# wwang2/CoarseGrainingVAE

Hardware: AMD Instinct MI355X
Metric: train_step_frames_per_sec (higher is better)
Workload: dtype f32

## Files before the change

### coarsegrainingvae_amd/_lib.py

```python
from __future__ import annotations

import ctypes as C
import os
import re
import threading

import torch

from . import ktimer

_PKG = os.path.dirname(os.path.abspath(__file__))
LIB_PATH = os.environ.get("CGV_LIB") or os.path.join(_PKG, "libcgvae_hip.so")
HEADER_PATH = os.path.join(os.path.dirname(_PKG), "include", "cgvae_hip.h")

_lock = threading.Lock()
_lib = None

_p, _i, _f, _sz = C.c_void_p, C.c_int, C.c_float, C.c_size_t

PROTOTYPES = {
    "cgv_version": (_i, []),
    "cgv_last_error_string": (C.c_char_p, []),
    "cgv_timestamp": (_i, [_p, _p]),
    "cgv_timestamp_hz": (_i, []),
# ... 17 lines not shown
    "cgv_edge_geometry_grouped": (_i, [_p, _p, _p, _p, _p, _i, _i, _f, _p, _p, _p]),
    "cgv_edge_geometry": (_i, [_p, _p, _p, _p, _p, _p, _i, _i, _f, _p, _p, _p]),
    "cgv_plan_jobs_max": (_i, []),
    "cgv_plan_job_bytes": (_i, []),
    "cgv_plan_jobs_build": (_i, [_p, _i, _p]),
    "cgv_geom_jobs_max": (_i, []),
    "cgv_geom_job_bytes": (_i, []),
    "cgv_geom_jobs_build": (_i, [_p, _i, _p]),
    "cgv_segment_reduce": (_i, [_p, _p, _p, _i, _i, _i, _p, _p]),
    "cgv_embedding_rows": (_i, [_p, _p, _i, _i, _i, _i, _p, _p]),
    "cgv_embedding_rows2": (_i, [_p, _p, _i, _i, _i, _p, _p, _p, _i, _i, _i, _p, _i, _p]),
    "cgv_segment_reduce_pair": (_i, [_p, _p, _p, _i, _p, _p, _p, _p, _i, _p, _i, _p]),
    "cgv_segment_broadcast": (_i, [_p, _p, _p, _i, _i, _i, _p, _p]),
    "cgv_equi_msg_fwd": (_i, [_p, _p, _p, _p, _p, _p, _p, _p, _p, _i, _i, _i, _i, C.c_int64, C.c_int64, _p, _p, _p]),
    "cgv_equi_msg_grouped_supported": (_i, [_i, _i, _i]),
    "cgv_equi_msg_fwd_grouped": (_i, [_p] * 9 + [_i, _i, _i, _i, C.c_int64, C.c_int64, _p, _p, _p]),
    "cgv_equi_msg_bwd_workspace_bytes": (_sz, [_i, _i, _i]),
    "cgv_equi_msg_bwd": (_i, [_p] * 13 + [_i, _i, _i, C.c_int64, C.c_int64, _p, _sz, _p]),
    "cgv_pseudo_msg_fwd": (_i, [_p] * 14 + [_i, _i, _i, _i, _p]),
    "cgv_pseudo_msg_fwd_rows": (_i, [_p] * 15 + [_i, _i, _i, _i, C.c_int64, _p]),
    "cgv_pseudo_msg_bwd_workspace_bytes": (_sz, [_i, _i, _i]),
    "cgv_pseudo_msg_bwd": (_i, [_p] * 24 + [_i, _i, _i, _i, C.c_int64, _p, _sz, _p]),
    "cgv_pseudo_msg_bwd_deferred": (_i, [_p] * 22 + [_i, _i, _i, _i, C.c_int64, _p, _sz, _p, _p]),
    "cgv_update_rows_from_vec": (_i, [_p, _p, _i, _i, _p]),
    "cgv_tile_bwd_input_plan": (_i, [_i, _i, _i, _i, _p, _p]),
    "cgv_tile_linear_bwd_input_norm_stack": (_i, [_p, _p, _p, _i, _i, _i, _i, _p, _p, _p, _p, _p, _i, _i, _p]),
    "cgv_update_vec_from_rows": (_i, [_p, _p, _p, _i, _i, _p]),
    "cgv_update_norm_stack_fwd": (_i, [_p, _p, _p, _i, _i, _i, _p]),
    "cgv_update_norm_stack_bwd": (_i, [_p, _p, _p, _p, _p, _p, _i, _i, _i, _i, _p]),
    "cgv_update_gate_fwd": (_i, [_p, _p, _p, _p, _p, _p, _p, _i, _i, _i, _p]),
    "cgv_update_gate_bwd": (_i, [_p, _p, _p, _p, _p, _p, _p, _p, _i, _i, _i, _p]),
    "cgv_skinny_max_rows": (_i, []),
    "cgv_skinny_supported": (_i, [_i, _i, _i]),
    "cgv_skinny_fwd_supported": (_i, [_i, _i, _i]),
    "cgv_skinny_linear_fwd": (_i, [_p, _p, _p, _p, _p, _i, _i, _i, _i, _p]),
    "cgv_skinny_bwd_input_supported": (_i, [_i, _i, _i]),
    "cgv_skinny_bwd_input_workspace_bytes": (_sz, [_i, _i, _i]),
    "cgv_skinny_linear_bwd_input": (_i, [_p, _p, _p, _p, _i, _i, _i, _i, _p, _sz, _p]),
    "cgv_decoder_layer_supported": (_i, [_i, _i, _i]),
    "cgv_decoder_slice_floats": (C.c_int64, [_i, _i]),
    "cgv_batch_load_rows": (_i, [_p, _p, _p, _i, _p, _p, _p, _i, _p]),
    "cgv_reparam_sample": (_i, [_p, _p, _p, _p, C.c_int64, _p, _p]),
    "cgv_reparam_bwd": (_i, [_p, _p, _p, _p, _p, _p, C.c_int64, _p]),
    "cgv_pair_linear_fwd": (_i, [_p] * 10 + [_i] * 5 + [_p]),
    "cgv_equi_msg_bwd_deferred": (_i, [_p] * 11 + [_i, _i, _i, C.c_int64, C.c_int64, _p, C.c_size_t, _p, _p, _p]),
    "cgv_filter_reduce_jobs_max": (_i, []),
    "cgv_filter_reduce_job_bytes": (_i, []),
    "cgv_filter_reduce_jobs": (_i, [_p, _i, _p]),
    "cgv_pair_linear_bwd_input": (_i, [_p] * 6 + [_i, _i, _p, _p, _i, _i, _i, _p, C.c_size_t, _p]),
    "cgv_loss_tail_supported": (_i, [_i, _i, _i, _i]),
    "cgv_loss_tail_workspace_bytes": (_sz, [_i]),
    "cgv_loss_tail": (_i, [_p] * 12 + [_i, _i, _i, _i, _i, _f, _f] + [_p] * 9 + [_p, _sz, _p]),
    "cgv_multi_linear_max": (_i, []),
    "cgv_multi_linear_fwd": (_i, [_i] + [_p] * 6 + [_i, _i, _i, _p]),
    "cgv_multi_linear_bwd_input": (_i, [_i, _i] + [_p] * 5 + [_i, _i, _i, _p, C.c_size_t, _p]),
    "cgv_decoder_max_edges": (_i, []),
    "cgv_decoder_block_channels": (_i, [_i]),
    "cgv_decoder_debug_clock": (_i, [_p]),
    "cgv_decoder_msg_fwd": (_i, [_p] * 18 + [_i, _i, _i, _i, _p]),
    "cgv_decoder_dense_fwd": (_i, [_p, _p, _p, _p, _p, _i, _i, _i, _i, _p]),
    "cgv_prior_msg_fwd": (_i, [_p] * 13 + [_i, _i, _i, _i, _i, _p]),
    "cgv_prior_msg_bwd": (_i, [_p] * 8 + [_i, C.c_int64] + [_p] * 6 + [C.c_int64, _i, _i, _i, _i, _p]),
    "cgv_decoder_uv_fwd": (_i, [_p, _p, _p, _p, _i, _i, _p]),
    "cgv_decoder_gate_fwd": (_i, [_p] * 9 + [_i, _i, _p]),
    "cgv_decoder_gate_bwd": (_i, [_p, _p, _p, _p, _i, C.c_int64, _p, _p, _p, _p, _p, _p, C.c_int64, _i, _i, _p]),
    "cgv_decoder_dense_bwd": (_i, [_p, _i, C.c_int64, _p, _i, _p, _p, _p, C.c_int64, _i, _i, _i, _p]),
    "cgv_decoder_uv_bwd": (_i, [_p, _i, C.c_int64, _p, _p, _p, _p, _p, _p, _p, _p, C.c_int64, _i, _i, _p]),
    "cgv_decoder_msg_bwd": (_i, [_p] * 15 + [_p, _i, C.c_int64, _p, _p, _p] + [_p] * 8 + [C.c_int64, _i, _i, _i, _i, _p]),
    "cgv_decoder_slices_to_dense": (_i, [_p, _p, _i, C.c_int64, _p, _i, _i, _p]),
    "cgv_dense_grad_prepare": (_i, [_p, _p, _p, _p, _i, _i, _i, _i, _p]),
    "cgv_tile_supported": (_i, [_i, _i, _i]),
    "cgv_tile_linear_fwd": (_i, [_p, _p, _p, _p, _p, _i, _i, _i, _i, _p]),
    "cgv_tile_linear_bwd_input": (_i, [_p, _p, _p, _i, _i, _i, _p]),
    "cgv_tile_linear_bwd_input_act": (_i, [_p, _p, _p, _p, _i, _i, _i, _i, _p]),
    "cgv_tile_linear_bwd_input_act_add": (_i, [_p, _p, _p, _p, _p, _i, _i, _i, _i, _p]),
    "cgv_tile_linear_bwd_input_act_add_bcast": (_i, [_p] * 7 + [_i, _p, _i, _i, _i, _i, _p]),
    "cgv_tile_pair_supported": (_i, [_i, _i, _i]),
    "cgv_tile_pair_linear_fwd": (_i, [_p] * 10 + [_i, _i, _i, _i, _i, _p]),
    "cgv_tile_pair_linear_bwd_input": (_i, [_p] * 10 + [_i, _i, _i, _i, _i, _p]),
    "cgv_tile_linear_bwd_input_out": (_i, [_p] * 5 + [_i, _i, _i, _i, _p, _i, _p]),
    "cgv_tile_bwd_input_split": (_i, [_p, _sz, _p]),
    "cgv_tile_pair_linear_bwd_input_out": (_i, [_p] * 10 + [_i, _i, _i, _i, _i, _p, _i, _p, _i, _p]),
    "cgv_tile_linear_bwd_input_sum2": (_i, [_p] * 10 + [_i, _p, _i, _i, _i, _i, _i, _p]),
    "cgv_segment_reduce2": (_i, [_p, _i, _p, _p, _i, _p, _p, _p, _i, _i, _p]),
    "cgv_skinny_linear_bwd_input_add": (_i, [_p, _p, _p, _p, _p, _i, _i, _i, _i, _p, _sz, _p]),
    "cgv_skinny_linear_bwd_input_out": (_i, [_p] * 5 + [_i, _i, _i, _i, _p, _i, _p, _sz, _p]),
    "cgv_tile_linear_wgrad": (_i, [_p, _p, _p, _i, _i, _i, _i, _p]),
    "cgv_wgrad_record_bytes": (_i, []),
    "cgv_wgrad_plan": (_i, [_i, _i, _i, _p, _p, _p]),
    "cgv_wgrad_lds_floats": (_i, [_i, _i]),
    "cgv_grouped_wgrad": (_i, [_p, _i, _i, _i, _p]),
    "cgv_wgrad_gathered_plan": (_i, [_i, _i, _i, _i, _p, _p]),
    "cgv_grouped_wgrad_gathered": (_i, [_p, _i, _i, _p]),
    "cgv_wgrad_gathered_plan_tile": (_i, [_i, _i, _i, _i, _i, _p, _p]),
    "cgv_grouped_wgrad_gathered_tile": (_i, [_p, _i, _i, _i, _p]),
    "cgv_grouped_wgrad_split": (_i, [_p, _i, _i, _p]),
    "cgv_grouped_wgrad_gathered_sumsq": (_i, [_p, _i, _i, _p, _p, _p]),
    "cgv_grouped_wgrad_gathered_adam": (_i, [_p, _i, _i, _p, _p, _p, _p, _f, _f, _f, _f, _p, _p]),
    "cgv_wgrad_strip_max_rows": (_i, []),
    "cgv_wgrad_strip_plan": (_i, [_i, _i, _i, _i, _p]),
    "cgv_wgrad_strip_split_max_rows": (_i, []),
    "cgv_wgrad_strip_split_plane_bytes": (_sz, [_i, _i]),
    "cgv_grouped_wgrad_strip_split": (_i, [_p, _i, _i, _i, _i, _p, _sz, _p]),
    "cgv_grouped_wgrad_strip": (_i, [_p, _i, _i, _i, _p]),
    "cgv_grouped_wgrad_strip_sumsq": (_i, [_p, _i, _i, _i, _p, _p, _p]),
    "cgv_grouped_wgrad_strip_adam": (_i, [_p, _i, _i, _i, _p, _p, _p, _p, _f, _f, _f, _f, _p, _p]),
    "cgv_pack_record_bytes": (_i, []),
    "cgv_pack_plan": (_i, [_i, _i, _i, _p]),
    "cgv_pack_operands": (_i, [_p, _i, _i, _p]),
    "cgv_reconstruct_fwd": (_i, [_p, _p, _p, _p, _p, _i, _i, _i, _p, _p]),
    "cgv_reconstruct_bwd": (_i, [_p, _p, _p, _p, _i, _i, _i, _p, _p, _p]),
    "cgv_elbo_workspace_bytes": (_sz, [_i, _i]),
    "cgv_elbo_fwd": (_i, [_p] * 7 + [_i, _i, _i, _i, _f, _f] + [_p] * 7 + [_p, _sz, _p]),
    "cgv_elbo_scale": (_i, [_p, _p, _p, _p, _p, _i, _p, _i, _p]),
    "cgv_optim_state_floats": (_i, []),
    "cgv_optim_partial_floats": (_i, []),
    "cgv_adam_clip_step": (_i, [_p, _p, _p, _p, C.c_int64, _f, _f, _f, _f, _f, _f, _p, _f, _p, _p, _p]),
    "cgv_optim_prepare": (_i, [_p, C.c_int64, _f, _f, _f, _f, _p, _f, _p, _p, _p]),
    "cgv_adam_apply": (_i, [_p, _p, _p, _p, C.c_int64, _f, _f, _f, _f, _p, _p]),
    "cgv_sgd_apply": (_i, [_p, _p, C.c_int64, _f, _p, _p]),
    "cgv_wgrad_gram": (_i, [_p, _i, _i, _p, _p, C.c_size_t, _p]),
    "cgv_wgrad_gram_workspace_bytes": (C.c_size_t, [_i]),
    "cgv_wgrad_gram_mfma": (_i, [_p, _i, _i, _p, _p, C.c_size_t, _p]),
    "cgv_wgrad_gram_mfma_workspace_bytes": (C.c_size_t, [_i, _i]),
    "cgv_wgrad_gram_mfma_max_rows": (_i, []),
    "cgv_rank_update_supported": (_i, [_i, _i, _i]),
    "cgv_optim_prepare_extra": (_i, [_p, C.c_int64, _p, _i, _f, _f, _f, _f, _p, _f, _p, _p, _p]),
    "cgv_grouped_wgrad_adam": (_i, [_p, _i, _i, _i, _p, _p, _p, _p, _f, _f, _f, _f, _p, _p]),
    "cgv_rank_flat_quantum": (_i, []),
    "cgv_rank_flat_plan": (_i, [_i, _i, _i, _i, _p, _p]),
    "cgv_grouped_wgrad_adam_flat": (_i, [_p, _i, _i, _i, _i, _p, _p, _p, _p, _f, _f, _f, _f, _p, _p]),
    "cgv_grouped_wgrad_adam_mixed": (_i, [_p, _i, _i, _i, _i, _i, _i, _p, _p, _p, _p, _f, _f, _f, _f, _p, _p]),
    "cgv_sample_quality_max_classes": (_i, []),
    "cgv_sample_quality": (_i, [_p] * 6 + [_i] * 5 + [_p, _p, _p]),
    "cgv_ensemble_check_max_classes": (_i, []),
    "cgv_ensemble_check_max_samples": (_i, []),
    "cgv_ensemble_check": (_i, [_p] * 7 + [_i] * 6 + [_p, _p, _p]),
    "cgv_internal_hist_max_features": (_i, []),
    "cgv_internal_hist_max_pairs": (_i, []),
    "cgv_internal_hist_max_bins": (_i, []),
    "cgv_internal_hist_max_bins2": (_i, []),
    "cgv_internal_hist_max_atoms": (_i, []),
    "cgv_internal_hist_max_staged_atoms": (_i, []),
    "cgv_internal_hist_feature_tile": (_i, [_i]),
    "cgv_internal_hist_pair_tile": (_i, [_i]),
    "cgv_internal_hist": (_i, [_p] * 4 + [_i] * 6 + [C.c_double] * 2 + [_p] * 3),
    "cgv_internal_values": (_i, [_p] * 3 + [_i] * 3 + [_p] * 3),
    "cgv_kde_max_planes": (_i, []),
    "cgv_kde_max_samples": (_i, []),
    "cgv_kde_max_points": (_i, []),
    "cgv_kde_max_splits": (_i, []),
    "cgv_kde_splits": (_i, [_i, _i, _i]),
    "cgv_kde_workspace_bytes": (_sz, [_i, _i, _i]),
    "cgv_kde_sums": (_i, [_p] * 3 + [_i] * 5 + [_p, _p, _p, _sz, _p]),
    "cgv_tica_max_features": (_i, []),
    "cgv_tica_max_atoms": (_i, []),
    "cgv_tica_max_bins2": (_i, []),
    "cgv_tica_max_components": (_i, []),
    "cgv_tica_moments_splits": (_i, [_i, _i, _i]),
    "cgv_tica_moments_workspace_bytes": (_sz, [_i, _i, _i]),
    "cgv_tica_moments": (_i, [_p, _p, _i, _i, _i, _i] + [_p] * 5 + [_p, _sz, _p]),
    "cgv_tica_project": (_i, [_p] * 4 + [_i] * 4 + [_p, _i, _i, _i] + [C.c_double] * 4 + [_p] * 3),
    "cgv_superpose_max_structures": (_i, []),
    "cgv_superpose_max_atoms": (_i, []),
    "cgv_superpose_workspace_bytes": (_sz, [_i, _i]),
    "cgv_superpose": (_i, [_p, _p, _p] + [_i] * 7 + [_p] * 5 + [_p, _sz, _p]),
# ... 108 lines not shown


def load():
    global _lib
    if _lib is not None:
        return _lib
    with _lock:
        if _lib is not None:
            return _lib
        if not os.path.exists(LIB_PATH):
            raise RuntimeError(
                f"{LIB_PATH} is missing: build it with `python -m coarsegrainingvae_amd.build` "
                "(hipcc --offload-arch=gfx950).  There is no fallback path.")
        lib = C.CDLL(LIB_PATH)
        for name, (res, args) in PROTOTYPES.items():
            fn = getattr(lib, name)
            fn.restype = res
            fn.argtypes = args
        if lib.cgv_version() < 101:
            raise RuntimeError("libcgvae_hip.so is older than this package")
        _lib = lib
    return _lib


def stream_ptr() -> int:
    return torch.cuda.current_stream().cuda_stream


def ptr(t):
    if t is None:
        return None
    if not t.is_cuda:
        raise RuntimeError("coarsegrainingvae_amd kernels need device (hip) tensors; there is no CPU path")
    if not t.is_contiguous():
        raise RuntimeError("tensor handed to the C ABI must be contiguous")
    return t.data_ptr()


_SPLIT_WS = {}
_SPLIT_TLS = threading.local()
_SPLIT_BYTES = 64 * 1024 + 64 * 1024 * 1024


def prepare_split_workspace(stream=None):
    st = torch.cuda.current_stream() if stream is None else stream
    key = (st.device.index if st.device.index is not None else torch.cuda.current_device(), int(st.cuda_stream))
    if key not in _SPLIT_WS:
        if torch.cuda.is_current_stream_capturing():
            return None
        _SPLIT_WS[key] = torch.zeros(_SPLIT_BYTES, dtype=torch.uint8, device=f"cuda:{key[0]}")
    return _SPLIT_WS[key]


def split_workspace_ready() -> bool:
    if load().cgv_get_option(OPTIONS["bwd_input_split"]) == 1:
        return False
    key = (torch.cuda.current_device(), int(torch.cuda.current_stream().cuda_stream))
    return key in _SPLIT_WS or not torch.cuda.is_current_stream_capturing()


def _register_split_workspace(lib):
    key = (torch.cuda.current_device(), int(torch.cuda.current_stream().cuda_stream))
    if getattr(_SPLIT_TLS, "cur", None) == key:
        return
    ws = prepare_split_workspace()
    if ws is None:
        lib.cgv_tile_bwd_input_split(None, 0, key[1])
        _SPLIT_TLS.cur = None
        return
    if lib.cgv_tile_bwd_input_split(ws.data_ptr(), ws.numel(), key[1]) != 0:
        raise RuntimeError("cgv_tile_bwd_input_split failed: " + lib.cgv_last_error_string().decode("utf-8", "replace"))
    _SPLIT_TLS.cur = key


def call(name: str, *args, tag=None):
    lib = load()
    if name.startswith("cgv_tile_") and ("bwd_input" in name or "linear_fwd" in name):
        _register_split_workspace(lib)
    tok = ktimer.begin(tag) if tag is not None else None
    rc = getattr(lib, name)(*args)
    ktimer.end(tok)
    if rc != 0:
        msg = lib.cgv_last_error_string().decode("utf-8", "replace")
        raise RuntimeError(f"{name} failed with code {rc}: {msg}")
```

### coarsegrainingvae_amd/csrc/tile_gemm.hip

```cpp
#include <stdlib.h>
#include <initializer_list>
#include <type_traits>
#include "cgv_common.h"
#include "streamk_gemm.h"

namespace cgv {

typedef float f32x4 __attribute__((ext_vector_type(4)));

__device__ __forceinline__ float4 ld4z(const float* p, bool ok) {
  return ok ? *reinterpret_cast<const float4*>(p) : make_float4(0.f, 0.f, 0.f, 0.f);
}

#define CGV_MFMA(a, b, c) __builtin_amdgcn_mfma_f32_16x16x4f32((a), (b), (c), 0, 0, 0)

template <int I0, int N, typename F>
__device__ __forceinline__ void static_for(F&& f) {
  if constexpr (I0 < N) {
    f(std::integral_constant<int, I0>{});
    static_for<I0 + 1, N>(f);
  }
}

struct TileSecond { const float* x; const float* W; const float* bias; float* y; float* z; int act; };
// ... 298 lines not shown
  __shared__ __attribute__((aligned(16))) float As[2][LT * LLD];
  __shared__ __attribute__((aligned(16))) float Bs[2][LT * LLD];
  const int t = threadIdx.x, lane = t & 63;
  const int wave = __builtin_amdgcn_readfirstlane(t >> 6);
  const int i = lane & 15, q = lane >> 4;
  const int wm = wave >> 1, wn = wave & 1;
  const int m0 = blockIdx.y * LT, n0 = blockIdx.x * LT;
  const int sr = t >> 3, sc = 4 * (t & 7);
  const float* const xr0 = x + (size_t)min(m0 + sr, M - 1) * K + sc;
  const float* const xr1 = x + (size_t)min(m0 + sr + 32, M - 1) * K + sc;
  const float* const wr0 = W + (size_t)min(n0 + sr, N - 1) * K + sc;
  const float* const wr1 = W + (size_t)min(n0 + sr + 32, N - 1) * K + sc;
  auto fetch = [&](RingSlot& r, int kt) __attribute__((always_inline)) {
    const int k0 = kt * LBK;
    const int off = (k0 + sc < K) ? k0 : -sc;
    r.a0 = *reinterpret_cast<const f32x4*>(xr0 + off); r.a1 = *reinterpret_cast<const f32x4*>(xr1 + off);
    r.b0 = *reinterpret_cast<const f32x4*>(wr0 + off); r.b1 = *reinterpret_cast<const f32x4*>(wr1 + off);
  };
  auto stash = [&](const RingSlot& r, int kt, int buf) __attribute__((always_inline)) {
    const bool kok = kt * LBK + sc < K;
    *reinterpret_cast<f32x4*>(&As[buf][sr * LLD + sc]) = r.a0;
    *reinterpret_cast<f32x4*>(&As[buf][(sr + 32) * LLD + sc]) = r.a1;
    *reinterpret_cast<f32x4*>(&Bs[buf][sr * LLD + sc]) = kok ? r.b0 : f32x4{0.f, 0.f, 0.f, 0.f};
    *reinterpret_cast<f32x4*>(&Bs[buf][(sr + 32) * LLD + sc]) = kok ? r.b1 : f32x4{0.f, 0.f, 0.f, 0.f};
  };
  RingSlot s0, s1, s2;
  fetch(s0, 0);
  fetch(s1, SLABS > 1 ? 1 : 0);
  fetch(s2, SLABS > 2 ? 2 : 0);
  f32x4 acc00 = {0.f, 0.f, 0.f, 0.f}, acc01 = acc00, acc10 = acc00, acc11 = acc00;
  stash(s0, 0, 0);
  __syncthreads();
#pragma unroll
  for (int kt = 0; kt < SLABS; ++kt) {
    const int buf = kt & 1;
    if (kt + 3 < SLABS) {
      switch (kt % 3) { case 0: fetch(s0, kt + 3); break; case 1: fetch(s1, kt + 3); break; default: fetch(s2, kt + 3); break; }
    }
    const float* __restrict__ a_s = As[buf] + (32 * wm + i) * LLD + 4 * q;
    const float* __restrict__ b_s = Bs[buf] + (32 * wn + i) * LLD + 4 * q;
#pragma unroll
    for (int ks = 0; ks < LBK / 16; ++ks) {
      const float4 x0 = *reinterpret_cast<const float4*>(a_s + 16 * ks), x1 = *reinterpret_cast<const float4*>(a_s + 16 * LLD + 16 * ks);
      const float4 w0 = *reinterpret_cast<const float4*>(b_s + 16 * ks), w1 = *reinterpret_cast<const float4*>(b_s + 16 * LLD + 16 * ks);
      acc00 = CGV_MFMA(w0.x, x0.x, acc00); acc01 = CGV_MFMA(w0.x, x1.x, acc01);
      acc10 = CGV_MFMA(w1.x, x0.x, acc10); acc11 = CGV_MFMA(w1.x, x1.x, acc11);
      acc00 = CGV_MFMA(w0.y, x0.y, acc00); acc01 = CGV_MFMA(w0.y, x1.y, acc01);
      acc10 = CGV_MFMA(w1.y, x0.y, acc10); acc11 = CGV_MFMA(w1.y, x1.y, acc11);
      acc00 = CGV_MFMA(w0.z, x0.z, acc00); acc01 = CGV_MFMA(w0.z, x1.z, acc01);
      acc10 = CGV_MFMA(w1.z, x0.z, acc10); acc11 = CGV_MFMA(w1.z, x1.z, acc11);
      acc00 = CGV_MFMA(w0.w, x0.w, acc00); acc01 = CGV_MFMA(w0.w, x1.w, acc01);
      acc10 = CGV_MFMA(w1.w, x0.w, acc10); acc11 = CGV_MFMA(w1.w, x1.w, acc11);
    }
    if (kt + 1 < SLABS) {
      switch ((kt + 1) % 3) { case 0: stash(s0, kt + 1, buf ^ 1); break; case 1: stash(s1, kt + 1, buf ^ 1); break; default: stash(s2, kt + 1, buf ^ 1); break; }
      __syncthreads();
    }
  }
  const f32x4 acc[2][2] = {{acc00, acc01}, {acc10, acc11}};
#pragma unroll
  for (int a = 0; a < 2; ++a) {
    const int n = n0 + 32 * wn + 16 * a + 4 * q;
    if (n >= N) continue;
    const float4 bv = bias ? *reinterpret_cast<const float4*>(bias + n) : make_float4(0.f, 0.f, 0.f, 0.f);
#pragma unroll
    for (int b = 0; b < 2; ++b) {
      const int m = m0 + 32 * wm + 16 * b + i;
      if (m >= M) continue;
      float4 zv = make_float4(acc[a][b][0] + bv.x, acc[a][b][1] + bv.y, acc[a][b][2] + bv.z, acc[a][b][3] + bv.w);
      if (act) {
        if (zout) *reinterpret_cast<float4*>(zout + (size_t)m * N + n) = zv;
        zv.x = act_fwd(zv.x, act); zv.y = act_fwd(zv.y, act); zv.z = act_fwd(zv.z, act); zv.w = act_fwd(zv.w, act);
      }
      *reinterpret_cast<float4*>(y + (size_t)m * N + n) = zv;
    }
  }
}

struct BwdSource { const float* g; const float* W; const float* z; int act; };
struct BwdSecond { const float* g; const float* W; float* gx; const float* z; const float* add; int act; };
struct OutAct { const float* z; int act; const float* z2; int act2; };
struct SplitN { float* part; unsigned* ticket; int n; };
struct NormStackOut { const float* stack; const float* Vv; const float* g_res; float* g_s; float* gVv; int F; int ld; int accumulate; };
struct BcastAdd {
  const float* src;
  const int64_t* row2seg;
  const int* rowptr;
  int mean;
};

#ifndef CGV_BWD_INPUT_PIPELINE
#define CGV_BWD_INPUT_PIPELINE 0
#endif
template <int MB, int WAVES>
__global__ __launch_bounds__(64 * WAVES) void tile_bwd_input_k(const float* __restrict__ g, const float* __restrict__ W,
                                                        float* __restrict__ gx, int M, int N, int K,
                                                        const float* __restrict__ z, int act,
                                                        const float* __restrict__ add = nullptr,
                                                        BcastAdd bc = BcastAdd{nullptr, nullptr, nullptr, 0},
                                                        BwdSecond s2 = BwdSecond{nullptr, nullptr, nullptr, nullptr, nullptr, 0},
                                                        BwdSource more = BwdSource{nullptr, nullptr, nullptr, 0},
                                                        OutAct oa = OutAct{nullptr, 0, nullptr, 0},
                                                        SplitN sp = SplitN{nullptr, nullptr, 1},
                                                        NormStackOut ns = NormStackOut{nullptr, nullptr, nullptr, nullptr, nullptr, 0, 0, 0}) {
  if (blockIdx.z) { g = s2.g; W = s2.W; gx = s2.gx; z = s2.z; add = s2.add; act = s2.act; bc.src = nullptr; oa.z = oa.z2; oa.act = oa.act2; }
  __shared__ float red[WAVES][MB * 4][4][64];
  const int lane = threadIdx.x & 63;
  const int wave = __builtin_amdgcn_readfirstlane(threadIdx.x >> 6);
  const int j = lane & 15, q = lane >> 4;
  const int ry = (int)blockIdx.y / sp.n, zs = (int)blockIdx.y - ry * sp.n;
  const int k0 = blockIdx.x * 64, m0 = ry * (16 * MB);
  const int kcol = k0 + 4 * j;
  const bool kok = kcol < K;
  const float* gr[MB];
  bool gok[MB];
#pragma unroll
  for (int mb = 0; mb < MB; ++mb) {
    const int m = m0 + 16 * mb + j;
    gok[mb] = m < M;
    gr[mb] = g + (size_t)(gok[mb] ? m : 0) * N + 4 * q;
  }
  const ptrdiff_t zoff = act ? z - g : 0;
  f32x4 acc[MB][4];
#pragma unroll
  for (int mb = 0; mb < MB; ++mb)
#pragma unroll
    for (int s = 0; s < 4; ++s) acc[mb][s] = f32x4{0.f, 0.f, 0.f, 0.f};
  const int steps_all = (N + 15) / 16, zper = (steps_all + sp.n - 1) / sp.n;
  const int z_beg = min(zs * zper, steps_all), steps = min(z_beg + zper, steps_all);
  const int per = (steps - z_beg + WAVES - 1) / WAVES;
  const int st_beg = min(z_beg + wave * per, steps), st_end = min(st_beg + per, steps);
  constexpr int SB = WAVES >= 16 ? 3 : 2;
  const float* wcol = W + (kok ? kcol : 0);
  ptrdiff_t zo = zoff;
  const int n_src = more.g ? 2 : 1;
  for (int src = 0; src < n_src; ++src) {
  if (src == 1) {
#pragma unroll
    for (int mb = 0; mb < MB; ++mb) gr[mb] = more.g + (gr[mb] - g);
    act = more.act;
    zo = act ? more.z - more.g : 0;
    wcol = more.W + (kok ? kcol : 0);
  }
  struct Batch { float4 a[SB][MB], zz[SB][MB], b[SB][4]; };
  auto request = [&](Batch& B, int st0) __attribute__((always_inline)) {
#pragma unroll
    for (int u = 0; u < SB; ++u) {
      const int n = 16 * (st0 + u);
      const bool in = st0 + u < st_end && n + 4 * q < N;
      const int ng = in ? n : -4 * q, nw = in ? n + 4 * q : 0;
#pragma unroll
      for (int mb = 0; mb < MB; ++mb) {
        B.a[u][mb] = *reinterpret_cast<const float4*>(gr[mb] + ng);
        if (act) B.zz[u][mb] = *reinterpret_cast<const float4*>(gr[mb] + zo + ng);
      }
#pragma unroll
      for (int c = 0; c < 4; ++c) B.b[u][c] = *reinterpret_cast<const float4*>(wcol + (size_t)(nw + c) * K);
    }
  };
  auto multiply = [&](const Batch& B, int st0) __attribute__((always_inline)) {
#pragma unroll
    for (int u = 0; u < SB; ++u) {
      if (st0 + u >= st_end) break;
      const bool nok = 16 * (st0 + u) + 4 * q < N;
#pragma unroll
      for (int mb = 0; mb < MB; ++mb) {
        float4 av = B.a[u][mb];
        if (act) {
          av.x *= act_bwd(B.zz[u][mb].x, act); av.y *= act_bwd(B.zz[u][mb].y, act);
          av.z *= act_bwd(B.zz[u][mb].z, act); av.w *= act_bwd(B.zz[u][mb].w, act);
        }
        const float ac[4] = {nok ? av.x : 0.f, nok ? av.y : 0.f, nok ? av.z : 0.f, nok ? av.w : 0.f};
#pragma unroll
        for (int c = 0; c < 4; ++c) {
          acc[mb][0] = CGV_MFMA(ac[c], B.b[u][c].x, acc[mb][0]);
          acc[mb][1] = CGV_MFMA(ac[c], B.b[u][c].y, acc[mb][1]);
          acc[mb][2] = CGV_MFMA(ac[c], B.b[u][c].z, acc[mb][2]);
          acc[mb][3] = CGV_MFMA(ac[c], B.b[u][c].w, acc[mb][3]);
        }
      }
    }
  };
  if constexpr (CGV_BWD_INPUT_PIPELINE && WAVES < 16) {
    Batch b0, b1;
    int st0 = st_beg;
    request(b0, st0);
    for (; st0 < st_end; st0 += 2 * SB) {
      request(b1, st0 + SB);
      multiply(b0, st0);
      request(b0, st0 + 2 * SB);
      multiply(b1, st0 + SB);
    }
  } else {
    for (int st0 = st_beg; st0 < st_end; st0 += SB) {
      Batch b0;
      request(b0, st0);
      multiply(b0, st0);
    }
  }
  }
  constexpr int PAIRS = MB * 4, PER = (PAIRS + WAVES - 1) / WAVES;
  float4 pre_add[PER], pre_z[PER];
  if (kok && (add || oa.z)) {
#pragma unroll
    for (int u = 0; u < PER; ++u) {
      const int c = wave + u * WAVES;
      if (c < PAIRS) {
        const size_t at = (size_t)min(m0 + 16 * (c >> 2) + 4 * q + (c & 3), M - 1) * K + kcol;
        if (add) pre_add[u] = *reinterpret_cast<const float4*>(add + at);
        if (oa.z) pre_z[u] = *reinterpret_cast<const float4*>(oa.z + at);
      }
    }
  }
#pragma unroll
  for (int t = 0; t < MB * 4; ++t)
#pragma unroll
    for (int r = 0; r < 4; ++r) red[wave][t][r][lane] = acc[t >> 2][t & 3][r];
  __syncthreads();
  float* tile_part = nullptr;
  if (sp.n > 1) {
    unsigned* s_last = reinterpret_cast<unsigned*>(&red[0][0][0][0]);
    const size_t tid = ((size_t)blockIdx.z * (gridDim.y / sp.n) + ry) * gridDim.x + blockIdx.x;
    tile_part = sp.part + tid * sp.n * (size_t)(MB * 16 * 64);
#pragma unroll
    for (int u = 0; u < PER; ++u) {
      const int c = wave + u * WAVES;
      if (c >= PAIRS) break;
      const int mb = c >> 2, r = c & 3;
      f32x4 o;
#pragma unroll
      for (int sI = 0; sI < 4; ++sI) {
        const int t = mb * 4 + sI;
        float a = red[0][t][r][lane];
#pragma unroll
        for (int w = 1; w < WAVES; ++w) a += red[w][t][r][lane];
        o[sI] = a;
      }
      float* dst = tile_part + (size_t)zs * (MB * 16 * 64) + (16 * mb + 4 * q + r) * 64 + 4 * j;
      asm volatile("global_store_dwordx4 %0, %1, off sc1" : : "v"(dst), "v"(o) : "memory");
    }
    asm volatile("s_waitcnt vmcnt(0)" ::: "memory");
    __syncthreads();
    if (threadIdx.x == 0) *s_last = atomicAdd(sp.ticket + tid, 1u) == (unsigned)(sp.n - 1) ? 1u : 0u;
    __syncthreads();
    if (!*s_last) return;
    if (threadIdx.x == 0) __hip_atomic_store(sp.ticket + tid, 0u, __ATOMIC_RELAXED, __HIP_MEMORY_SCOPE_AGENT);
  }
// ... 201 lines not shown
                       act);
  else if (lds_min == 5)
    hipLaunchKernelGGL((cgv::tile_fwd_k<1, 2, 8>), dim3((N + 63) / 64, (M + 31) / 32), dim3(1024), 0, st, x, W, bias, y, z, M, N, K, act);
  else if (lds_min == 6)
    hipLaunchKernelGGL((cgv::tile_fwd_k<2, 1, 8>), dim3((N + 31) / 32, (M + 63) / 64), dim3(1024), 0, st, x, W, bias, y, z, M, N, K, act);
  else if (lds_min == 7)
    hipLaunchKernelGGL((cgv::tile_fwd_k<2, 2, 4>), dim3((N + 63) / 64, (M + 63) / 64), dim3(1024), 0, st, x, W, bias, y, z, M, N, K, act);
  else if (tiles32 >= 2048)
    hipLaunchKernelGGL((cgv::tile_fwd_k<2, 2, 4>), dim3((N + 63) / 64, (M + 63) / 64, np), dim3(1024), 0, st, x, W, bias, y, z, M,
                       N, K, act, s2);
  else
    hipLaunchKernelGGL((cgv::tile_fwd_k<1, 1, 8>), dim3((N + 31) / 32, (M + 31) / 32, np), dim3(512), 0, st, x, W, bias, y, z, M,
                       N, K, act, s2);
  return cgv::check_launch("cgv_tile_linear_fwd");
}

int cgv_tile_linear_fwd(const float* x, const float* W, const float* bias, float* y, float* z, int M, int N, int K, int act,
                        void* stream) {
  CGV_REQUIRE(x && W && y, "null pointer");
  CGV_REQUIRE(act >= 0 && act <= cgv::CGV_ACT_MAX, "act must be 0 (identity), 1 (swish), 2 (tanh), 3 (relu), 4 / 5 (c + exp(z/2))");
  CGV_REQUIRE(cgv_tile_supported(M, N, K), "unsupported shape (need N % 4 == 0, K % 4 == 0)");
  CGV_REQUIRE(((((uintptr_t)x | (uintptr_t)W)) & 15) == 0, "x and W must be 16-byte aligned");
  return tile_fwd_launch(x, W, bias, y, z, M, N, K, act, stream, nullptr);
}

int cgv_tile_pair_supported(int M, int N, int K) {
  return cgv_tile_supported(M, N, K);
}

int cgv_tile_pair_linear_fwd(const float* x_a, const float* W_a, const float* bias_a, float* y_a, float* z_a, const float* x_b,
                             const float* W_b, const float* bias_b, float* y_b, float* z_b, int M, int N, int K, int act_a,
                             int act_b, void* stream) {
  const int act = act_a;
  CGV_REQUIRE(x_a && W_a && y_a && x_b && W_b && y_b, "null pointer");
  CGV_REQUIRE(act_a >= 0 && act_a <= cgv::CGV_ACT_MAX && act_b >= 0 && act_b <= cgv::CGV_ACT_MAX,
              "act must be 0 (identity), 1 (swish), 2 (tanh), 3 (relu), 4 / 5 (c + exp(z/2))");
  CGV_REQUIRE((act_a == 0 || z_a) && (act_b == 0 || z_b), "act != 0 needs the pre-activation output");
  CGV_REQUIRE(cgv_tile_supported(M, N, K), "unsupported shape (need N % 4 == 0, K % 4 == 0)");
  CGV_REQUIRE(((((uintptr_t)x_a | (uintptr_t)W_a | (uintptr_t)x_b | (uintptr_t)W_b | (uintptr_t)y_a | (uintptr_t)y_b |
                 (uintptr_t)z_a | (uintptr_t)z_b | (uintptr_t)bias_a | (uintptr_t)bias_b)) & 15) == 0, "operands must be 16-byte aligned");
  const cgv::TileSecond s2{x_b, W_b, bias_b, y_b, z_b, act_b};
  return tile_fwd_launch(x_a, W_a, bias_a, y_a, z_a, M, N, K, act, stream, &s2);
}


static int split_shares(int tiles, int N) {
  const int opt = cgv::option(CGV_OPT_BWD_INPUT_SPLIT);
  if (opt == 1 || tiles > 128 || tiles < 1) return 1;
  int n = opt >= 2 ? opt : 256 / tiles;
  n = n > 4 ? 4 : n;
  while (n > 1 && (N + 15) / 16 / n < 16) --n;
  return n < 1 ? 1 : n;
}

namespace cgv {
enum BwdKernel { BWD_R16_W8, BWD_R16_W16, BWD_R32_W8, BWD_R32_W4 };
struct BwdInputChoice {
  int bpc;
  BwdKernel kernel;
  int shares;
};

static BwdInputChoice bwd_input_choice(int M, int N, int K, int np, bool ws) {
  BwdInputChoice c{ws ? sk_wanted(M, K, N, np) : 0, BWD_R16_W8, 1};
  const int kt = (K + 63) / 64;
  const int blocks32 = kt * ((M + 31) / 32);
  const int blocks16 = kt * ((M + 15) / 16);
  const int ow = option(CGV_OPT_BWD_INPUT_WAVES);
  int waves = 8;
  if (ow > 0 && ow != 32) waves = ow;
  else if (blocks16 < 128 && N >= 1024) waves = 16;
  if (ow == 32 || (blocks32 >= 200 && blocks32 < 512 && waves == 8))
    c.kernel = BWD_R32_W8;
  else if (blocks32 >= 512)
    c.kernel = BWD_R32_W4;
  else if (waves == 16) {
    c.kernel = BWD_R16_W16;
    if (ws) c.shares = split_shares(blocks16 * np, N);
  }
  return c;
}
}

static int tile_bwd_input_launch(const float* g, const float* z, int act, const float* W, float* gx, int M, int N, int K,
                                 void* stream, const char* what, const float* add = nullptr,
                                 cgv::BcastAdd bc = cgv::BcastAdd{nullptr, nullptr, nullptr, 0},
                                 const cgv::BwdSecond* second = nullptr,
                                 cgv::BwdSource more = cgv::BwdSource{nullptr, nullptr, nullptr, 0},
                                 cgv::OutAct oa = cgv::OutAct{nullptr, 0, nullptr, 0},
                                 cgv::NormStackOut ns = cgv::NormStackOut{nullptr, nullptr, nullptr, nullptr, nullptr, 0, 0, 0}) {
  hipStream_t st = (hipStream_t)stream;
  const cgv::BwdSecond s2 = second ? *second : cgv::BwdSecond{nullptr, nullptr, nullptr, nullptr, nullptr, 0};
  const unsigned np = second ? 2u : 1u;
  const cgv::BwdInputChoice choice = cgv::bwd_input_choice(M, N, K, (int)np, cgv::sk_ws_ready(stream));
  if (const int bpc = choice.bpc;
      bpc != 0 && !ns.stack && act == 0 && (!more.g || more.act == 0) && (!second || s2.act == 0) &&
      cgv::sk_aligned({g, W, gx, add, bc.src, more.g, more.W, oa.z, oa.z2, s2.g, s2.W, s2.gx, s2.add})) {
    cgv::SkArgs a{};
    a.np = (int)np; a.M = M; a.N = K;
    cgv::SkProblem& p0 = a.p[0];
    p0.A[0] = g; p0.B[0] = W; p0.R[0] = N; p0.out = gx; p0.add = add;
    if (more.g) { p0.A[1] = more.g; p0.B[1] = more.W; p0.R[1] = N; }
    p0.bc_src = bc.src; p0.bc_row2seg = bc.row2seg; p0.bc_rowptr = bc.rowptr; p0.bc_mean = bc.mean;
    p0.oz = oa.z; p0.oact = oa.act;
    if (second) {
      cgv::SkProblem& p1 = a.p[1];
      p1.A[0] = s2.g; p1.B[0] = s2.W; p1.R[0] = N; p1.out = s2.gx; p1.add = s2.add; p1.oz = oa.z2; p1.oact = oa.act2;
    }
    if (cgv::sk_launch(a, true, cgv::g_split_ws.ws, cgv::g_split_ws.bytes, cgv::SPLIT_TICKET_BYTES, st, bpc) == 0)
      return cgv::check_launch(what);
  }
  const int kt = (K + 63) / 64;
  switch (choice.kernel) {
    case cgv::BWD_R32_W8:
      hipLaunchKernelGGL((cgv::tile_bwd_input_k<2, 8>), dim3(kt, (M + 31) / 32, np), dim3(512), 0, st, g, W, gx, M, N, K, z, act, add, bc, s2, more, oa, cgv::SplitN{nullptr, nullptr, 1}, ns);
      break;
    case cgv::BWD_R32_W4:
      hipLaunchKernelGGL((cgv::tile_bwd_input_k<2, 4>), dim3(kt, (M + 31) / 32, np), dim3(256), 0, st, g, W, gx, M, N, K, z, act, add, bc, s2, more, oa, cgv::SplitN{nullptr, nullptr, 1}, ns);
      break;
    case cgv::BWD_R16_W16: {
      cgv::SplitN sp{nullptr, nullptr, 1};
      const int tiles = kt * ((M + 15) / 16) * (int)np;
      const cgv::SplitWs& w = cgv::g_split_ws;
      const size_t need = cgv::SPLIT_TICKET_BYTES + (size_t)tiles * choice.shares * (16 * 64) * sizeof(float);
      if (choice.shares > 1 && need <= w.bytes && (size_t)tiles * sizeof(unsigned) <= cgv::SPLIT_TICKET_BYTES) {
        sp.ticket = reinterpret_cast<unsigned*>(w.ws);
        sp.part = reinterpret_cast<float*>(reinterpret_cast<char*>(w.ws) + cgv::SPLIT_TICKET_BYTES);
        sp.n = choice.shares;
      }
      hipLaunchKernelGGL((cgv::tile_bwd_input_k<1, 16>), dim3(kt, ((M + 15) / 16) * sp.n, np), dim3(1024), 0, st, g, W, gx, M, N, K, z, act,
                         add, bc, s2, more, oa, sp, ns);
      break;
    }
    case cgv::BWD_R16_W8:
      hipLaunchKernelGGL((cgv::tile_bwd_input_k<1, 8>), dim3(kt, (M + 15) / 16, np), dim3(512), 0, st, g, W, gx, M, N, K, z, act, add, bc, s2, more, oa, cgv::SplitN{nullptr, nullptr, 1}, ns);
      break;
  }
  return cgv::check_launch(what);
}

int cgv_tile_bwd_input_plan(int M, int N, int K, int np, int* shares, int* streamk) {
  CGV_REQUIRE(shares && streamk && np >= 1 && np <= 2, "bad argument");
  CGV_REQUIRE(cgv_tile_supported(M, N, K), "unsupported shape (need N % 4 == 0, K % 4 == 0)");
  const cgv::BwdInputChoice c = cgv::bwd_input_choice(M, N, K, np, true);
  *streamk = c.bpc != 0;
  *shares = c.bpc != 0 ? 1 : c.shares;
  return 0;
}

int cgv_tile_bwd_input_split(void* ws, size_t bytes, void* stream) {
  CGV_REQUIRE(!ws || ((((uintptr_t)ws) & 15) == 0 && bytes >= cgv::SPLIT_TICKET_BYTES + (2u << 20)), "workspace too small / misaligned");
  cgv::g_split_ws = cgv::SplitWs{ws, ws ? bytes : 0, stream};
  return 0;
}

int cgv_tile_linear_bwd_input(const float* g, const float* W, float* gx, int M, int N, int K, void* stream) {
  CGV_REQUIRE(g && W && gx, "null pointer");
  CGV_REQUIRE(cgv_tile_supported(M, N, K), "unsupported shape (need N % 4 == 0, K % 4 == 0)");
  CGV_REQUIRE(((((uintptr_t)g | (uintptr_t)W | (uintptr_t)gx)) & 15) == 0, "g, W and gx must be 16-byte aligned");
  return tile_bwd_input_launch(g, nullptr, 0, W, gx, M, N, K, stream, "cgv_tile_linear_bwd_input");
}

int cgv_tile_linear_bwd_input_act(const float* gy, const float* z, const float* W, float* gx, int M, int N, int K, int act,
                                  void* stream) {
  CGV_REQUIRE(gy && W && gx, "null pointer");
  CGV_REQUIRE(act == 0 || (act >= 1 && act <= cgv::CGV_ACT_MAX && z), "act != 0 needs the saved pre-activation z");
  CGV_REQUIRE(cgv_tile_supported(M, N, K), "unsupported shape (need N % 4 == 0, K % 4 == 0)");
  CGV_REQUIRE(((((uintptr_t)gy | (uintptr_t)z | (uintptr_t)W | (uintptr_t)gx)) & 15) == 0, "operands must be 16-byte aligned");
  return tile_bwd_input_launch(gy, act ? z : nullptr, act, W, gx, M, N, K, stream, "cgv_tile_linear_bwd_input_act");
}

int cgv_tile_linear_bwd_input_act_add(const float* gy, const float* z, const float* W, const float* add, float* gx, int M, int N,
                                      int K, int act, void* stream) {
  CGV_REQUIRE(gy && W && gx && add, "null pointer");
  CGV_REQUIRE(act == 0 || (act >= 1 && act <= cgv::CGV_ACT_MAX && z), "act != 0 needs the saved pre-activation z");
  CGV_REQUIRE(cgv_tile_supported(M, N, K), "unsupported shape (need N % 4 == 0, K % 4 == 0)");
  CGV_REQUIRE(((((uintptr_t)gy | (uintptr_t)z | (uintptr_t)W | (uintptr_t)gx | (uintptr_t)add)) & 15) == 0, "operands must be 16-byte aligned");
  return tile_bwd_input_launch(gy, act ? z : nullptr, act, W, gx, M, N, K, stream, "cgv_tile_linear_bwd_input_act_add", add);
}

int cgv_tile_linear_bwd_input_act_add_bcast(const float* gy, const float* z, const float* W, const float* add, const float* seg_grad,
                                            const int64_t* row2seg, const int32_t* seg_rowptr, int mean, float* gx, int M, int N,
                                            int K, int act, void* stream) {
  CGV_REQUIRE(gy && W && gx && seg_grad && row2seg && seg_rowptr, "null pointer");
  CGV_REQUIRE(act == 0 || (act >= 1 && act <= cgv::CGV_ACT_MAX && z), "act != 0 needs the saved pre-activation z");
  CGV_REQUIRE(cgv_tile_supported(M, N, K), "unsupported shape (need N % 4 == 0, K % 4 == 0)");
  CGV_REQUIRE(((((uintptr_t)gy | (uintptr_t)z | (uintptr_t)W | (uintptr_t)gx | (uintptr_t)add | (uintptr_t)seg_grad)) & 15) == 0,
              "operands must be 16-byte aligned");
  return tile_bwd_input_launch(gy, act ? z : nullptr, act, W, gx, M, N, K, stream, "cgv_tile_linear_bwd_input_act_add_bcast", add,
                               cgv::BcastAdd{seg_grad, row2seg, seg_rowptr, mean});
}

int cgv_tile_linear_bwd_input_sum2(const float* gy_a, const float* z_a, const float* W_a, const float* gy_b, const float* z_b,
                                   const float* W_b, const float* add, const float* seg_grad, const int64_t* row2seg,
                                   const int32_t* seg_rowptr, int mean, float* gx, int M, int N, int K, int act_a, int act_b,
                                   void* stream) {
  CGV_REQUIRE(gy_a && W_a && gy_b && W_b && gx, "null pointer");
  CGV_REQUIRE((act_a == 0 || (act_a >= 1 && act_a <= cgv::CGV_ACT_MAX && z_a)) && (act_b == 0 || (act_b >= 1 && act_b <= cgv::CGV_ACT_MAX && z_b)),
              "act != 0 needs the saved pre-activation");
  CGV_REQUIRE(!seg_grad || (row2seg && seg_rowptr), "seg_grad needs its row -> segment map and the segments' row pointers");
  CGV_REQUIRE(cgv_tile_supported(M, N, K), "unsupported shape (need N % 4 == 0, K % 4 == 0)");
  CGV_REQUIRE(((((uintptr_t)gy_a | (uintptr_t)z_a | (uintptr_t)W_a | (uintptr_t)gy_b | (uintptr_t)z_b | (uintptr_t)W_b | (uintptr_t)gx |
                 (uintptr_t)add | (uintptr_t)seg_grad)) & 15) == 0, "operands must be 16-byte aligned");
  return tile_bwd_input_launch(gy_a, act_a ? z_a : nullptr, act_a, W_a, gx, M, N, K, stream, "cgv_tile_linear_bwd_input_sum2", add,
                               cgv::BcastAdd{seg_grad, row2seg, seg_rowptr, mean}, nullptr,
                               cgv::BwdSource{gy_b, W_b, act_b ? z_b : nullptr, act_b});
}

int cgv_tile_pair_linear_bwd_input(const float* gy_a, const float* z_a, const float* W_a, const float* add_a, float* gx_a,
                                   const float* gy_b, const float* z_b, const float* W_b, const float* add_b, float* gx_b, int M,
                                   int N, int K, int act_a, int act_b, void* stream) {
  const int act = act_a;
  CGV_REQUIRE(gy_a && W_a && gx_a && gy_b && W_b && gx_b && gx_a != gx_b, "null pointer / aliased outputs");
  CGV_REQUIRE((act_a == 0 || (act_a >= 1 && act_a <= cgv::CGV_ACT_MAX && z_a)) && (act_b == 0 || (act_b >= 1 && act_b <= cgv::CGV_ACT_MAX && z_b)),
              "act != 0 needs the saved pre-activation");
  CGV_REQUIRE(cgv_tile_supported(M, N, K), "unsupported shape (need N % 4 == 0, K % 4 == 0)");
  CGV_REQUIRE(((((uintptr_t)gy_a | (uintptr_t)z_a | (uintptr_t)W_a | (uintptr_t)gx_a | (uintptr_t)add_a | (uintptr_t)gy_b |
                 (uintptr_t)z_b | (uintptr_t)W_b | (uintptr_t)gx_b | (uintptr_t)add_b)) & 15) == 0, "operands must be 16-byte aligned");
  const cgv::BwdSecond s2{gy_b, W_b, gx_b, act_b ? z_b : nullptr, add_b, act_b};
  return tile_bwd_input_launch(gy_a, act ? z_a : nullptr, act, W_a, gx_a, M, N, K, stream, "cgv_tile_pair_linear_bwd_input", add_a,
                               cgv::BcastAdd{nullptr, nullptr, nullptr, 0}, &s2);
}

int cgv_tile_linear_bwd_input_out(const float* gy, const float* z, const float* W, const float* add, float* gx, int M, int N,
                                  int K, int act, const float* z_out, int act_out, void* stream) {
  CGV_REQUIRE(gy && W && gx && z_out, "null pointer");
  CGV_REQUIRE(act == 0 || (act >= 1 && act <= cgv::CGV_ACT_MAX && z), "act != 0 needs the saved pre-activation z");
  CGV_REQUIRE(act_out >= 1 && act_out <= cgv::CGV_ACT_MAX, "act_out must name an activation");
  CGV_REQUIRE(cgv_tile_supported(M, N, K), "unsupported shape (need N % 4 == 0, K % 4 == 0)");
  CGV_REQUIRE(((((uintptr_t)gy | (uintptr_t)z | (uintptr_t)W | (uintptr_t)gx | (uintptr_t)add | (uintptr_t)z_out)) & 15) == 0,
              "operands must be 16-byte aligned");
  return tile_bwd_input_launch(gy, act ? z : nullptr, act, W, gx, M, N, K, stream, "cgv_tile_linear_bwd_input_out", add,
                               cgv::BcastAdd{nullptr, nullptr, nullptr, 0}, nullptr, cgv::BwdSource{nullptr, nullptr, nullptr, 0},
                               cgv::OutAct{z_out, act_out, nullptr, 0});
}

int cgv_tile_linear_bwd_input_norm_stack(const float* gy, const float* z, const float* W, int M, int N, int K, int act,
                                         const float* stack, const float* Vv, const float* g_res, float* g_s, float* gVv, int ld,
                                         int accumulate, void* stream) {
  CGV_REQUIRE(gy && W && stack && Vv && g_s && gVv, "null pointer");
  CGV_REQUIRE(act == 0 || (act >= 1 && act <= cgv::CGV_ACT_MAX && z), "act != 0 needs the saved pre-activation z");
  CGV_REQUIRE(cgv_tile_supported(M, N, K) && K % 8 == 0 && ld >= K / 2 && ld % 4 == 0, "unsupported shape (need K = 2 F, F % 4 == 0, ld % 4 == 0)");
  CGV_REQUIRE(((((uintptr_t)gy | (uintptr_t)z | (uintptr_t)W | (uintptr_t)stack | (uintptr_t)Vv | (uintptr_t)g_res | (uintptr_t)g_s |
                 (uintptr_t)gVv)) & 15) == 0, "operands must be 16-byte aligned");
  return tile_bwd_input_launch(gy, act ? z : nullptr, act, W, g_s , M, N, K, stream,
                               "cgv_tile_linear_bwd_input_norm_stack", nullptr, cgv::BcastAdd{nullptr, nullptr, nullptr, 0}, nullptr,
                               cgv::BwdSource{nullptr, nullptr, nullptr, 0}, cgv::OutAct{nullptr, 0, nullptr, 0},
                               cgv::NormStackOut{stack, Vv, g_res, g_s, gVv, K / 2, ld, accumulate});
}

int cgv_tile_pair_linear_bwd_input_out(const float* gy_a, const float* z_a, const float* W_a, const float* add_a, float* gx_a,
                                       const float* gy_b, const float* z_b, const float* W_b, const float* add_b, float* gx_b,
                                       int M, int N, int K, int act_a, int act_b, const float* z_out_a, int act_out_a,
                                       const float* z_out_b, int act_out_b, void* stream) {
  const int act = act_a;
  CGV_REQUIRE(gy_a && W_a && gx_a && gy_b && W_b && gx_b && gx_a != gx_b, "null pointer / aliased outputs");
  CGV_REQUIRE((act_a == 0 || (act_a >= 1 && act_a <= cgv::CGV_ACT_MAX && z_a)) && (act_b == 0 || (act_b >= 1 && act_b <= cgv::CGV_ACT_MAX && z_b)),
              "act != 0 needs the saved pre-activation");
  CGV_REQUIRE((!z_out_a || (act_out_a >= 1 && act_out_a <= cgv::CGV_ACT_MAX)) && (!z_out_b || (act_out_b >= 1 && act_out_b <= cgv::CGV_ACT_MAX)),
              "z_out needs its activation code");
  CGV_REQUIRE(cgv_tile_supported(M, N, K), "unsupported shape (need N % 4 == 0, K % 4 == 0)");
  CGV_REQUIRE(((((uintptr_t)gy_a | (uintptr_t)z_a | (uintptr_t)W_a | (uintptr_t)gx_a | (uintptr_t)add_a | (uintptr_t)gy_b |
                 (uintptr_t)z_b | (uintptr_t)W_b | (uintptr_t)gx_b | (uintptr_t)add_b | (uintptr_t)z_out_a | (uintptr_t)z_out_b)) & 15) == 0,
              "operands must be 16-byte aligned");
  const cgv::BwdSecond s2{gy_b, W_b, gx_b, act_b ? z_b : nullptr, add_b, act_b};
  return tile_bwd_input_launch(gy_a, act ? z_a : nullptr, act, W_a, gx_a, M, N, K, stream, "cgv_tile_pair_linear_bwd_input_out", add_a,
                               cgv::BcastAdd{nullptr, nullptr, nullptr, 0}, &s2, cgv::BwdSource{nullptr, nullptr, nullptr, 0},
                               cgv::OutAct{z_out_a, z_out_a ? act_out_a : 0, z_out_b, z_out_b ? act_out_b : 0});
}

int cgv_tile_linear_wgrad(const float* g, const float* x, float* gW, int M, int N, int K, int accumulate, void* stream) {
  CGV_REQUIRE(g && x && gW, "null pointer");
  CGV_REQUIRE(cgv_tile_supported(M, N, K), "unsupported shape (need N % 4 == 0, K % 4 == 0)");
  CGV_REQUIRE(((((uintptr_t)x | (uintptr_t)gW)) & 15) == 0, "x and gW must be 16-byte aligned");
  const dim3 grid((K + 63) / 64, (N + 15) / 16);
  if (grid.x * grid.y >= 1024 || M <= 128)
    hipLaunchKernelGGL((cgv::tile_wgrad_k<4>), grid, dim3(256), 0, (hipStream_t)stream, g, x, gW, M, N, K, accumulate);
  else
    hipLaunchKernelGGL((cgv::tile_wgrad_k<8>), grid, dim3(512), 0, (hipStream_t)stream, g, x, gW, M, N, K, accumulate);
  return cgv::check_launch("cgv_tile_linear_wgrad");
}

}
```

### coarsegrainingvae_amd/csrc/wgrad_gathered.hip

```cpp
#include "cgv_common.h"
#include "gemm_dev.h"
#include "wgrad_record.h"

namespace cgv {

__device__ __forceinline__ float4 ldg4_or_zero(const float* p, bool ok) {
  return ok ? *reinterpret_cast<const float4*>(p) : make_float4(0.f, 0.f, 0.f, 0.f);
}
__device__ __forceinline__ void strip_pin() { asm volatile("" ::: "memory"); }
typedef const float __attribute__((address_space(1)))* strip_gptr;
__device__ __forceinline__ float4 strip_ldg4(const float* p) {
  const f32x4 t = *reinterpret_cast<const __attribute__((address_space(1))) f32x4*>((strip_gptr)p);
  return make_float4(t.x, t.y, t.z, t.w);
}
#ifndef CGV_GW_CHUNK
#define CGV_GW_CHUNK 48
#endif
constexpr int GW_CHUNK = CGV_GW_CHUNK;
constexpr int GW_GS = 80, GW_XS = 64;
constexpr int GW_TW = 128, GW_XW = 128;

enum { GW_STORE = 0, GW_SUMSQ = 1, GW_ADAM = 2 };
template <int MODE>
__global__ __launch_bounds__(256) void gathered_wgrad_k(const WgradProblem* __restrict__ table, int n_problems,
// ... 433 lines not shown
#pragma unroll
    for (int p = 0; p < NP; ++p) {
      *reinterpret_cast<float4*>(gs + (rr + 8 * p) * GW2_GS + 4 * c4) = gq[p];
      *reinterpret_cast<float4*>(xs + (rr + 8 * p) * GW2_XS + 4 * c4) = xq[p];
    }
    __syncthreads();
    if (m0 + GW2_CHUNK < M) chunk_load(m0 + GW2_CHUNK);
    const int steps = (rows + 3) / 4;
#pragma unroll 2
    for (int st = 0; st < steps; ++st) {
      const float4 b = *reinterpret_cast<const float4*>(xs + (4 * st + q) * GW2_XS + 64 * wk + 4 * i);
#pragma unroll
      for (int t = 0; t < 4; ++t) {
        const float a = gs[(4 * st + q) * GW2_GS + 64 * wn + 16 * t + i];
        bsum[t] += a;
        acc[t][0] = __builtin_amdgcn_mfma_f32_16x16x4f32(a, b.x, acc[t][0], 0, 0, 0);
        acc[t][1] = __builtin_amdgcn_mfma_f32_16x16x4f32(a, b.y, acc[t][1], 0, 0, 0);
        acc[t][2] = __builtin_amdgcn_mfma_f32_16x16x4f32(a, b.z, acc[t][2], 0, 0, 0);
        acc[t][3] = __builtin_amdgcn_mfma_f32_16x16x4f32(a, b.w, acc[t][3], 0, 0, 0);
      }
    }
    __syncthreads();
  }
  const int kcol = k0 + 64 * wk + 4 * i;
  if (kcol < K) {
#pragma unroll
    for (int t = 0; t < 4; ++t)
#pragma unroll
      for (int r = 0; r < 4; ++r) {
        const int row = n0 + 64 * wn + 16 * t + 4 * q + r;
        if (row >= N) continue;
        float4* dst = reinterpret_cast<float4*>(pr.gW + (size_t)row * K + kcol);
        float4 o = make_float4(acc[t][0][r], acc[t][1][r], acc[t][2][r], acc[t][3][r]);
        if (pr.accumulate) { const float4 old = *dst; o.x += old.x; o.y += old.y; o.z += old.z; o.w += old.w; }
        *dst = o;
      }
  }
  if (pr.gb && kt == 0 && wk == 0) {
#pragma unroll
    for (int t = 0; t < 4; ++t) {
      float b = bsum[t];
      b += __shfl_xor(b, 16);
      b += __shfl_xor(b, 32);
      const int n = n0 + 64 * wn + 16 * t + i;
      if (q == 0 && n < N) pr.gb[n] = pr.accumulate ? pr.gb[n] + b : b;
    }
  }
}

typedef __bf16 sp_bf16x2 __attribute__((ext_vector_type(2)));
typedef __bf16 sp_bf16x8 __attribute__((ext_vector_type(8)));
typedef float sp_f32x2 __attribute__((ext_vector_type(2)));
constexpr int SP_CHUNK = 32;
constexpr int SP_LD = 40;

__device__ __forceinline__ void sp_split(float a, float b, unsigned& hi, unsigned& mid, unsigned& lo) {
  const sp_f32x2 v = {a, b};
  const sp_bf16x2 h = __builtin_convertvector(v, sp_bf16x2);
  const sp_f32x2 r = v - __builtin_convertvector(h, sp_f32x2);
  const sp_bf16x2 m = __builtin_convertvector(r, sp_bf16x2);
  const sp_f32x2 r2 = r - __builtin_convertvector(m, sp_f32x2);
  const sp_bf16x2 l = __builtin_convertvector(r2, sp_bf16x2);
  hi = __builtin_bit_cast(unsigned, h);
  mid = __builtin_bit_cast(unsigned, m);
  lo = __builtin_bit_cast(unsigned, l);
}
__device__ __forceinline__ void sp_store4(unsigned short* dst, int plane, float v0, float v1, float v2, float v3) {
  unsigned h0, m0, l0, h1, m1, l1;
  sp_split(v0, v1, h0, m0, l0);
  sp_split(v2, v3, h1, m1, l1);
  *reinterpret_cast<uint2*>(dst) = make_uint2(h0, h1);
  *reinterpret_cast<uint2*>(dst + plane) = make_uint2(m0, m1);
  *reinterpret_cast<uint2*>(dst + 2 * plane) = make_uint2(l0, l1);
}

__global__ __launch_bounds__(256, 2) void wgrad_split128_k(const WgradProblem* __restrict__ table, int n_problems) {
  constexpr int PLANE = 128 * SP_LD;
  __shared__ __attribute__((aligned(16))) unsigned short gs[3 * PLANE];
  __shared__ __attribute__((aligned(16))) unsigned short xs[3 * PLANE];
  const int item = blockIdx.x;
  const int lo = wg_find_problem(table, n_problems, item);
  const WgradProblem pr = table[lo];
  const int local = item - pr.block_begin;
  const int nb = local / pr.tiles_k, kt = local - nb * pr.tiles_k;
  const int M = pr.M, N = pr.N, K = pr.K;
  const int sr = pr.seg_rows > 0 ? pr.seg_rows : M;
  const int n0 = nb * 128, k0 = kt * 128;
  const int lane = threadIdx.x & 63;
  const int wave = __builtin_amdgcn_readfirstlane(threadIdx.x >> 6);
  const int wn = wave >> 1, wk = wave & 1;
  const int i = lane & 15, q = lane >> 4;
  typedef float f32x4 __attribute__((ext_vector_type(4)));
  f32x4 acc[4][4];
#pragma unroll
  for (int t = 0; t < 4; ++t)
#pragma unroll
    for (int c = 0; c < 4; ++c) acc[t][c] = f32x4{0.f, 0.f, 0.f, 0.f};
  const int c4 = 8 * wave + (lane & 7), rq = lane >> 3;
  const bool gcol = n0 + 4 * c4 < N, xcol = k0 + 4 * c4 < K;
  const int gcol_at = gcol ? n0 + 4 * c4 : 0, xcol_at = xcol ? k0 + 4 * c4 : 0;
  const float* zsrc = pr.act ? pr.z : pr.gy;
  float4 gq[4], zq[4], xq[4];
  float bs[4] = {0.f, 0.f, 0.f, 0.f};
  auto chunk_load = [&](int m0) {
#pragma unroll
    for (int r = 0; r < 4; ++r) {
      const int m = min(m0 + 4 * rq + r, M - 1);
      const int seg = m / sr, row = m - seg * sr;
      const size_t base = (size_t)seg * pr.seg_stride;
      gq[r] = strip_ldg4(pr.gy + base + (size_t)row * N + gcol_at);
      zq[r] = strip_ldg4(zsrc + base + (size_t)row * N + gcol_at);
      xq[r] = strip_ldg4(pr.x + base + (size_t)row * K + xcol_at);
    }
    strip_pin();
  };
  unsigned short* gdst = gs + (4 * c4) * SP_LD + 4 * rq;
  unsigned short* xdst = xs + (64 * (c4 >> 4) + (c4 & 15)) * SP_LD + 4 * rq;
  auto chunk_store = [&](int m0) {
    if (pr.act == 1) {
#pragma unroll
      for (int r = 0; r < 4; ++r) {
        gq[r].x *= act_bwd(zq[r].x, 1); gq[r].y *= act_bwd(zq[r].y, 1);
        gq[r].z *= act_bwd(zq[r].z, 1); gq[r].w *= act_bwd(zq[r].w, 1);
      }
    } else if (pr.act) {
#pragma unroll
      for (int r = 0; r < 4; ++r) {
        gq[r].x *= act_bwd(zq[r].x, pr.act); gq[r].y *= act_bwd(zq[r].y, pr.act);
        gq[r].z *= act_bwd(zq[r].z, pr.act); gq[r].w *= act_bwd(zq[r].w, pr.act);
      }
    }
#pragma unroll
    for (int r = 0; r < 4; ++r) {
      const bool live = m0 + 4 * rq + r < M;
      if (!(live && gcol)) gq[r] = make_float4(0.f, 0.f, 0.f, 0.f);
      if (!(live && xcol)) xq[r] = make_float4(0.f, 0.f, 0.f, 0.f);
    }
    bs[0] += (gq[0].x + gq[1].x) + (gq[2].x + gq[3].x);
    bs[1] += (gq[0].y + gq[1].y) + (gq[2].y + gq[3].y);
    bs[2] += (gq[0].z + gq[1].z) + (gq[2].z + gq[3].z);
    bs[3] += (gq[0].w + gq[1].w) + (gq[2].w + gq[3].w);
    sp_store4(gdst, PLANE, gq[0].x, gq[1].x, gq[2].x, gq[3].x);
    sp_store4(gdst + SP_LD, PLANE, gq[0].y, gq[1].y, gq[2].y, gq[3].y);
    sp_store4(gdst + 2 * SP_LD, PLANE, gq[0].z, gq[1].z, gq[2].z, gq[3].z);
    sp_store4(gdst + 3 * SP_LD, PLANE, gq[0].w, gq[1].w, gq[2].w, gq[3].w);
    sp_store4(xdst, PLANE, xq[0].x, xq[1].x, xq[2].x, xq[3].x);
    sp_store4(xdst + 16 * SP_LD, PLANE, xq[0].y, xq[1].y, xq[2].y, xq[3].y);
    sp_store4(xdst + 32 * SP_LD, PLANE, xq[0].z, xq[1].z, xq[2].z, xq[3].z);
    sp_store4(xdst + 48 * SP_LD, PLANE, xq[0].w, xq[1].w, xq[2].w, xq[3].w);
  };
  const unsigned short* ga = gs + (64 * wn + i) * SP_LD + 8 * q;
  const unsigned short* xb = xs + (64 * wk + i) * SP_LD + 8 * q;
  chunk_load(0);
  for (int m0 = 0; m0 < M; m0 += SP_CHUNK) {
    chunk_store(m0);
    __syncthreads();
    chunk_load(min(m0 + SP_CHUNK, M - 1));
    sp_bf16x8 a[3][4];
#pragma unroll
    for (int s = 0; s < 3; ++s)
#pragma unroll
      for (int t = 0; t < 4; ++t) a[s][t] = *reinterpret_cast<const sp_bf16x8*>(ga + s * PLANE + 16 * t * SP_LD);
#pragma unroll
    for (int c = 0; c < 4; ++c) {
      sp_bf16x8 b[3];
#pragma unroll
      for (int s = 0; s < 3; ++s) b[s] = *reinterpret_cast<const sp_bf16x8*>(xb + s * PLANE + 16 * c * SP_LD);
#pragma unroll
      for (int t = 0; t < 4; ++t) acc[t][c] = __builtin_amdgcn_mfma_f32_16x16x32_bf16(a[0][t], b[2], acc[t][c], 0, 0, 0);
#pragma unroll
      for (int t = 0; t < 4; ++t) acc[t][c] = __builtin_amdgcn_mfma_f32_16x16x32_bf16(a[2][t], b[0], acc[t][c], 0, 0, 0);
#pragma unroll
      for (int t = 0; t < 4; ++t) acc[t][c] = __builtin_amdgcn_mfma_f32_16x16x32_bf16(a[1][t], b[1], acc[t][c], 0, 0, 0);
#pragma unroll
      for (int t = 0; t < 4; ++t) acc[t][c] = __builtin_amdgcn_mfma_f32_16x16x32_bf16(a[0][t], b[1], acc[t][c], 0, 0, 0);
#pragma unroll
      for (int t = 0; t < 4; ++t) acc[t][c] = __builtin_amdgcn_mfma_f32_16x16x32_bf16(a[1][t], b[0], acc[t][c], 0, 0, 0);
#pragma unroll
      for (int t = 0; t < 4; ++t) acc[t][c] = __builtin_amdgcn_mfma_f32_16x16x32_bf16(a[0][t], b[0], acc[t][c], 0, 0, 0);
    }
    __syncthreads();
  }
  const int kcol = k0 + 64 * wk + 4 * i;
// ... 415 lines not shown
```

### coarsegrainingvae_amd/csrc/wgrad_record.h

```cpp
#pragma once
#include "cgv_common.h"

namespace cgv {

struct WgradProblem {
  const float* gy;
  const float* x;
  const float* z;
  float* gW;
  float* gb;
  int M, N, K;
  int accumulate, act;
  int block_begin;
  int tiles_k;
  int tile_w;
  int seg_rows;
  int seg_stride;
  int pad;
};
static_assert(sizeof(WgradProblem) == 88, "host/device record layout");
__device__ __forceinline__ size_t wg_row(const WgradProblem& pr, int m, int width) {
  if (pr.seg_rows <= 0) return (size_t)m * width;
  const int seg = m / pr.seg_rows;
  return (size_t)seg * pr.seg_stride + (size_t)(m - seg * pr.seg_rows) * width;
}

template <typename Problem>
__device__ __forceinline__ int wg_find_problem(const Problem* __restrict__ table, int n_problems, int block) {
  const int lane = threadIdx.x & 63;
  int count = 0;
  for (int base = 0; base < n_problems; base += 64) {
    const int i = base + lane;
    const int bb = i < n_problems ? table[i].block_begin : 0x7fffffff;
    count += __popcll(__ballot(bb <= block));
  }
  return __builtin_amdgcn_readfirstlane(count > 0 ? count - 1 : 0);
}
template <typename Problem>
__device__ __forceinline__ int wg_find_problem(const Problem* __restrict__ table, int n_problems) {
  return wg_find_problem(table, n_problems, (int)blockIdx.x);
}

struct RankUpdateArgs {
  const float* arena_g;
  float* arena_p;
  float* arena_m;
  float* arena_v;
  const float* state;
  float lr, beta1, beta2, eps;
};

constexpr int GRAM_MAX_ROWS = 64;

}
```

### coarsegrainingvae_amd/ops.py

```python
from __future__ import annotations

from typing import Optional

import ctypes as C
from types import SimpleNamespace

import torch

from . import _lib, options
from .graph import EdgeGeometry, EdgePlan
from .primitives import FWD_ENTRY, bwd_input_choice, bwd_input_launch, fwd_choice, linear as _linear, wgrad_queue, wgrad_sink

_F32 = torch.float32


def _c(t: Optional[torch.Tensor]) -> Optional[torch.Tensor]:
    if t is None:
        return None
    if t.dtype != _F32:
        raise RuntimeError("the HIP path computes in fp32 only")
    return t.contiguous()


def _filter_grad_targets(params, Wd, bd):
    pW, pb = params
    direct = all(getattr(p, "_cgv_direct", False) and p.grad is not None and p._cgv_pending and p.grad.is_contiguous()
                 for p in (pW, pb))
    if direct:
        pW._cgv_pending = pb._cgv_pending = False
        return pW.grad, pb.grad, None, None
    gWd, gbd = torch.empty_like(Wd), torch.empty_like(bd)
    return gWd, gbd, gWd, gbd


def _grouped_forward_usable(plan, geom, F, tensors8, Wd) -> bool:
    if not getattr(plan, "group_rb", 0) or getattr(geom, "geom_g", None) is None or plan.n_edges == 0:
        return False
    if not _lib.load().cgv_equi_msg_grouped_supported(F, geom.n_rbf, plan.group_rb):
        return False
    if plan.n_src * 12 * F >= 0x7fffffff or Wd.data_ptr() % 16:
        return False
    return all(t is None or t.data_ptr() % 8 == 0 for t in tensors8)


class _EquiMessage(torch.autograd.Function):

    @staticmethod
    def forward(ctx, phi, v, Wd, bd, plan: EdgePlan, geom: EdgeGeometry, with_dv: bool, s_res, v_res):
        filter_params = (Wd, bd)
        phi, v, Wd, bd, s_res, v_res = _c(phi), _c(v), _c(Wd), _c(bd), _c(s_res), _c(v_res)
        ctx.residual = (s_res is not None, v_res is not None)
        F = phi.shape[1] // 3
        if phi.shape[0] != plan.n_src or v.shape != (plan.n_src, F, 3) or Wd.shape != (3 * F, geom.n_rbf):
            raise RuntimeError("shape mismatch between node features, filter weights and the edge plan")
        ds = torch.empty(plan.n_dst, F, dtype=_F32, device=phi.device)
        if with_dv:
            dv = torch.empty(plan.n_dst, F, 3, dtype=_F32, device=phi.device)
        else:
            dv = v_res.clone() if v_res is not None else torch.zeros(plan.n_dst, F, 3, dtype=_F32, device=phi.device)
        tag = f"equi_msg_fwd:Nd{plan.n_dst}:E{plan.n_edges}:dv{int(with_dv)}"
        grouped = with_dv and _grouped_forward_usable(plan, geom, F, (phi, v, ds, dv, s_res, v_res, bd), Wd)
        if grouped:
            _lib.call("cgv_equi_msg_fwd_grouped", _lib.ptr(phi), _lib.ptr(v), _lib.ptr(geom.geom_g), _lib.ptr(plan.rowptr_d),
                      _lib.ptr(plan.src_g), _lib.ptr(Wd), _lib.ptr(bd), _lib.ptr(ds), _lib.ptr(dv),
                      plan.n_dst, F, geom.n_rbf, plan.group_rb, plan.n_src, plan.n_edges, _lib.ptr(s_res), _lib.ptr(v_res),
                      _lib.stream_ptr(), tag=tag)
        else:
            _lib.call("cgv_equi_msg_fwd", _lib.ptr(phi), _lib.ptr(v), _lib.ptr(geom.geom_d), _lib.ptr(plan.rowptr_d),
                      _lib.ptr(plan.src_d), _lib.ptr(Wd), _lib.ptr(bd), _lib.ptr(ds), _lib.ptr(dv), plan.n_dst, F,
                      geom.n_rbf, int(with_dv), plan.n_edges, plan.n_src, _lib.ptr(s_res), _lib.ptr(v_res),
                      _lib.stream_ptr(), tag=tag)
        ctx.save_for_backward(phi, v, Wd, bd)
        ctx.filter_params = filter_params
        ctx.plan, ctx.geom, ctx.with_dv = plan, geom, with_dv
        ctx.set_materialize_grads(False)
        return ds, dv

    @staticmethod
    def backward(ctx, gs, gv):
        phi, v, Wd, bd = ctx.saved_tensors
        plan, geom = ctx.plan, ctx.geom
        F = phi.shape[1] // 3
        dev = phi.device
        g_sres = gs if ctx.residual[0] else None
        g_vres = gv if ctx.residual[1] else None
        if not ctx.with_dv:
            gv = None
        if gs is None and gv is None:
            return (None,) * 7 + (g_sres, g_vres)
        gs, gv = _c(gs), _c(gv)
        g_phi = torch.empty_like(phi)
        g_v = torch.empty_like(v) if gv is not None else None
        gWd, gbd, ret_W, ret_b = _filter_grad_targets(ctx.filter_params, Wd, bd)
        lib = _lib.load()
        ws_bytes = int(lib.cgv_equi_msg_bwd_workspace_bytes(plan.n_src, F, geom.n_rbf))
        ws = torch.empty(ws_bytes, dtype=torch.uint8, device=dev)
        if wgrad_queue.active and ret_W is None and ret_b is None:
            nc, kl = C.c_int(), C.c_int()
            _lib.call("cgv_equi_msg_bwd_deferred", _lib.ptr(phi), _lib.ptr(v), _lib.ptr(geom.geom_s), _lib.ptr(plan.rowptr_s),
                      _lib.ptr(plan.dst_s), _lib.ptr(Wd), _lib.ptr(bd), _lib.ptr(gs), _lib.ptr(gv), _lib.ptr(g_phi), _lib.ptr(g_v),
                      plan.n_src, F, geom.n_rbf, plan.n_edges, plan.n_dst, _lib.ptr(ws), ws_bytes, C.byref(nc), C.byref(kl),
                      _lib.stream_ptr(), tag=f"equi_msg_bwd:Nd{plan.n_dst}:E{plan.n_edges}:gv{int(gv is not None)}")
            wgrad_queue.enqueue_filter(ws, nc.value, kl.value, geom.n_rbf, F, gWd, gbd)
            return g_phi, g_v, ret_W, ret_b, None, None, None, g_sres, g_vres
        _lib.call("cgv_equi_msg_bwd", _lib.ptr(phi), _lib.ptr(v), _lib.ptr(geom.geom_s), _lib.ptr(plan.rowptr_s),
                  _lib.ptr(plan.dst_s), _lib.ptr(Wd), _lib.ptr(bd), _lib.ptr(gs), _lib.ptr(gv), _lib.ptr(g_phi),
                  _lib.ptr(g_v), _lib.ptr(gWd), _lib.ptr(gbd), plan.n_src, F, geom.n_rbf, plan.n_edges, plan.n_dst, _lib.ptr(ws), ws_bytes,
                  _lib.stream_ptr(), tag=f"equi_msg_bwd:Nd{plan.n_dst}:E{plan.n_edges}:gv{int(gv is not None)}")
        return g_phi, g_v, ret_W, ret_b, None, None, None, g_sres, g_vres


def equi_message(phi, v, Wd, bd, plan: EdgePlan, geom: EdgeGeometry, with_dv: bool = True, s_res=None, v_res=None):
    return _EquiMessage.apply(phi, v, Wd, bd, plan, geom, with_dv, s_res, v_res)


class _SegmentReduce(torch.autograd.Function):
    @staticmethod
    def forward(ctx, src, plan: EdgePlan, mean: bool):
        src = _c(src)
        rows = src.shape[0]
        if rows != plan.n_edges:
            raise RuntimeError("index plan and src disagree on the number of rows")
        flat = src.reshape(rows, -1)
        C = flat.shape[1]
        out = torch.empty((plan.n_dst, C), dtype=_F32, device=src.device)
        _lib.call("cgv_segment_reduce", _lib.ptr(flat), _lib.ptr(plan.rowptr_d), _lib.ptr(plan.eid_d), plan.n_dst, C,
                  int(mean), _lib.ptr(out), _lib.stream_ptr())
        ctx.plan, ctx.mean, ctx.shape = plan, mean, tuple(src.shape)
        ctx.set_materialize_grads(False)
        return out.reshape((plan.n_dst,) + tuple(src.shape[1:]))

    @staticmethod
    def backward(ctx, gout):
        if gout is None:
            return None, None, None
        plan = ctx.plan
        gout = _c(gout).reshape(plan.n_dst, -1)
        C = gout.shape[1]
        gsrc = torch.empty((plan.n_edges, C), dtype=_F32, device=gout.device)
        _lib.call("cgv_segment_broadcast", _lib.ptr(gout), _lib.ptr(plan.rowptr_d), _lib.ptr(plan.eid_d), plan.n_dst,
                  C, int(ctx.mean), _lib.ptr(gsrc), _lib.stream_ptr())
        return gsrc.reshape(ctx.shape), None, None


class _Embedding(torch.autograd.Function):

    @staticmethod
    def forward(ctx, weight, idx, plan: EdgePlan):
        ctx.plan, ctx.param = plan, weight
        if idx.dtype == torch.float32 and idx.dim() == 1 and weight.shape[1] % 4 == 0:
            out = torch.empty(idx.shape[0], weight.shape[1], dtype=_F32, device=weight.device)
            _lib.call("cgv_embedding_rows", _lib.ptr(weight.detach()), idx.data_ptr(), int(idx.stride(0)), idx.shape[0],
                      weight.shape[0], weight.shape[1], _lib.ptr(out), _lib.stream_ptr())
            return out
        return weight.index_select(0, idx.long())

    @staticmethod
    def backward(ctx, g):
        from .primitives import _grad_target
        plan, w = ctx.plan, ctx.param
        g = _c(g)
        n_types, F = w.shape
        target, accumulate, ret = _grad_target(w, w)
        out = torch.empty_like(target) if accumulate else target
        _lib.call("cgv_segment_reduce", _lib.ptr(g), _lib.ptr(plan.rowptr_d), _lib.ptr(plan.eid_d), n_types, F, 0,
                  _lib.ptr(out), _lib.stream_ptr())
        if accumulate:
            target.add_(out)
        return ret, None, None


class _Embedding2(torch.autograd.Function):

    @staticmethod
    def forward(ctx, w_a, idx_a, plan_a, w_b, idx_b, plan_b):
        F = w_a.shape[1]
        out_a = torch.empty(idx_a.shape[0], F, dtype=_F32, device=w_a.device)
        out_b = torch.empty(idx_b.shape[0], F, dtype=_F32, device=w_a.device)
        _lib.call("cgv_embedding_rows2", _lib.ptr(w_a.detach()), idx_a.data_ptr(), int(idx_a.stride(0)), idx_a.shape[0], w_a.shape[0],
                  _lib.ptr(out_a), _lib.ptr(w_b.detach()), idx_b.data_ptr(), int(idx_b.stride(0)), idx_b.shape[0], w_b.shape[0],
                  _lib.ptr(out_b), F, _lib.stream_ptr())
        ctx.plans, ctx.params = (plan_a, plan_b), (w_a, w_b)
        ctx.set_materialize_grads(False)
        return out_a, out_b

    @staticmethod
# ... 661 lines not shown
```

### coarsegrainingvae_amd/options.py

```python
from __future__ import annotations

from . import _lib

HOST = {
    "fwd_group": -1,
    "wgrad_kernel": 0,
    "table_upload": 0,
    "wgrad_tile": 64,
    "rank_update": 1,
    "rank_flat": 2,
    "rank_mixed": 1,
    "rank_rows_mfma": -1,
    "rank_gram_rows": -1,
    "concurrent_prior": 0,
    "quad_heads": 1,
    "fused_loss_tail": 1,
    "paired_embeddings": 1,
    "pair_sum2": 1,
    "head_pairs": 1,
    "encoder_pairs": 1,
    "wgrad_split": 1,
    "fused_bead_mean": 1,
    "fused_prior": 1,
    "act_downstream": 1,
    "update_fused_bwd": 1,
    "strip_split": 1,
    "cgae_form": 0,
    "newman_form": 0,
    "baseline_form": 0,
    "align_form": 0,
    "kde_splits": 0,
    "decoder_dense": 0,
}
_DEFAULTS = dict(HOST)


def set(name: str, value: int) -> None:
    if name in HOST:
        HOST[name] = int(value)
    elif name in _lib.OPTIONS:
        _lib.set_option(name, int(value))
    else:
        raise KeyError(f"unknown option {name!r}; known: {sorted(HOST) + sorted(_lib.OPTIONS)}")


def get(name: str) -> int:
    return HOST[name] if name in HOST else _lib.get_option(name)


def reset() -> None:
    HOST.update(_DEFAULTS)
    _lib.reset_options()


def apply(specs) -> None:
    for spec in specs or ():
        name, _, value = spec.partition("=")
        set(name.strip(), int(value))


def pop_cli(argv) -> list:
    rest, i = [], 0
    while i < len(argv):
        if argv[i] == "--option" and i + 1 < len(argv):
            apply([argv[i + 1]])
            i += 2
        else:
            rest.append(argv[i])
            i += 1
    return rest
```

### coarsegrainingvae_amd/primitives.py

```python
from __future__ import annotations

import ctypes as C
import struct

import numpy as np
import torch
import torch.nn.functional as Fn
from torch import nn

from . import _lib


class Swish(nn.Module):

    def forward(self, x):
        return Fn.silu(x)


class shifted_softplus(nn.Module):
    def forward(self, x):
        return Fn.softplus(x) - np.log(2.0)


layer_types = {
    "linear": nn.Linear, "Tanh": nn.Tanh, "ReLU": nn.ReLU, "shifted_softplus": shifted_softplus,
    "sigmoid": nn.Sigmoid, "Dropout": nn.Dropout, "LeakyReLU": nn.LeakyReLU, "ELU": nn.ELU, "swish": Swish,
}


def to_module(activation: str) -> nn.Module:
    return layer_types[activation]()


def gemm_mode_or_none(x2, weight, bias):
    if not (x2.is_cuda and weight.is_cuda):
        return None, ("Dense / Linear run on the HIP kernels only: move the module and its input to the device "
                      "(there is no CPU / library fallback)")
    if x2.dtype != torch.float32 or weight.dtype != torch.float32:
        return None, "the HIP path computes in fp32 only"
    if not (weight.is_contiguous() and weight.data_ptr() % 16 == 0):
        return None, "Dense / Linear: the weight must be contiguous and 16-byte aligned"
    M, K = x2.shape
    N = weight.shape[0]
    if M == 0:
        return None, f"Dense / Linear on an input without rows (0 x {K})"
    lib = _lib.load()
    if lib.cgv_skinny_supported(M, N, K) and (bias is None or bias.data_ptr() % 16 == 0):
        return "skinny", None
    if lib.cgv_tile_supported(M, N, K):
        return "tile", None
    return None, (f"Dense / Linear {M} x {N} x {K}: the HIP kernels take in / out widths that are multiples of 4 "
                  f"(other widths are zero-padded by primitives.linear_fn before they get here)")


def _gemm_mode(x2, weight, bias):
    mode, why = gemm_mode_or_none(x2, weight, bias)
    if mode is None:
        raise RuntimeError(why)
    return mode


ACT_NONE, ACT_SWISH, ACT_TANH, ACT_RELU = 0, 1, 2, 3
ACT_STD_ENC, ACT_STD_PRIOR = 4, 5
_STD_EPS = {ACT_STD_ENC: 1e-12, ACT_STD_PRIOR: 1e-9}


class WeightGradQueue:

    RECORD = struct.Struct("<5Q11i4x")
    MAX_PROBLEMS = 512

    def __init__(self):
        self.active = False
        self.items = []
        self._captured = []
        self._capture_slots = []
        self._deferred = []
        self.filters = []

    @property
    def kernel(self):
        from .options import HOST
        return "mfma" if HOST["wgrad_kernel"] == 1 else "valu"

    @property
    def static_tables(self):
        from .options import HOST
        return HOST["table_upload"] != 1

    def prepare_capture(self, device, flushes: int = 4):
        n = self.MAX_PROBLEMS * self.RECORD.size
        self._captured = []
        self._capture_slots = [(torch.empty(n, dtype=torch.uint8).pin_memory(),
                                torch.empty(n, dtype=torch.uint8, device=device)) for _ in range(flushes)]

    def collect(self):
        return _QueueScope(self)

    def enqueue(self, gy, x, z, act, gW, gb, accumulate):
        self.items.append((gy, x, z, act, gW, gb, accumulate))

    def take(self):
        items, self.items = self.items, []
        return items

    def flush(self):
        self.launch(self.take())
        self.flush_filters()

    def enqueue_filter(self, ws, n_chunks, k_live, n_rbf, F, gWd, gbd):
        self.filters.append((ws, int(n_chunks), int(k_live), int(n_rbf), int(F), gWd, gbd))

    def flush_filters(self):
        jobs, self.filters = self.filters, []
        if not jobs:
            return
        lib = _lib.load()

        class Job(C.Structure):
            _fields_ = [("part", C.c_void_p), ("gWd", C.c_void_p), ("gbd", C.c_void_p), ("n_chunks", C.c_int), ("K", C.c_int),
                        ("R", C.c_int), ("F", C.c_int)]
        assert C.sizeof(Job) == lib.cgv_filter_reduce_job_bytes()
        cap = int(lib.cgv_filter_reduce_jobs_max())
        for at in range(0, len(jobs), cap):
            part = jobs[at:at + cap]
            table = (Job * len(part))(*[Job(ws.data_ptr(), gW.data_ptr(), gb.data_ptr(), nc, k, r, f) for ws, nc, k, r, f, gW, gb in part])
            _lib.call("cgv_filter_reduce_jobs", C.addressof(table), len(part), _lib.stream_ptr(), tag="filter_reduce_jobs")

    def upload(self, buf: bytes, device):
        capturing = torch.cuda.is_current_stream_capturing()
        if capturing:
            if not self._capture_slots:
                raise RuntimeError("call wgrad_queue.prepare_capture(device) with enough slots before capturing a step")
            host, table = slot = self._capture_slots.pop()
            self._captured.append(slot)
        else:
            n = (len(buf) + 255) // 256 * 256
            host = torch.empty(n, dtype=torch.uint8, pin_memory=True)
            table = torch.empty(n, dtype=torch.uint8, device=device)
        if len(buf) > host.numel():
            raise RuntimeError("record table exceeds the staging buffer")
        host[: len(buf)].copy_(torch.frombuffer(bytearray(buf), dtype=torch.uint8))
        if capturing and self.static_tables:
            self._deferred.append((host, table, len(buf)))
        else:
            table[: len(buf)].copy_(host[: len(buf)], non_blocking=True)
        return table

    def finish_capture(self):
        for host, table, n in self._deferred:
            table[:n].copy_(host[:n], non_blocking=True)
        if self._deferred:
            torch.cuda.current_stream().synchronize()
        self._deferred = []
        used, self._captured, self._capture_slots = self._captured, [], []
        return used

    def small_table(self, items):
        lib = _lib.load()
        tk, tw, nb = C.c_int(), C.c_int(), C.c_int()
        buf, block_begin, max_lds = bytearray(), 0, 0
        for gy, x, z, act, gW, gb, accumulate in items:
            M, N = gy.shape
            K = x.shape[1]
            if lib.cgv_wgrad_plan(M, N, K, C.byref(tk), C.byref(tw), C.byref(nb)) != 0:
                raise RuntimeError(lib.cgv_last_error_string().decode())
            buf += self.RECORD.pack(gy.data_ptr(), x.data_ptr(), z.data_ptr() if z is not None else 0, gW.data_ptr(),
                                    gb.data_ptr() if gb is not None else 0, M, N, K, int(accumulate), int(act),
                                    block_begin, tk.value, tw.value, 0, 0, 0)
            block_begin += nb.value
            max_lds = max(max_lds, lib.cgv_wgrad_lds_floats(M, tw.value))
        return self.upload(bytes(buf), items[0][0].device), block_begin, max_lds

    def rank_table(self, items, q4=0):
        lib = _lib.load()
        q4 = int(lib.cgv_rank_flat_quantum()) if q4 == 0 else int(q4)
        nb, lds, tk, tw = C.c_int(), C.c_int(), C.c_int(), C.c_int()
        flat, tiled = [], []
        for it in items:
            M, N = it[0].shape
            ok = q4 > 0 and not it[6] and lib.cgv_rank_flat_plan(M, N, it[1].shape[1], q4, C.byref(nb), C.byref(lds)) == 0
            (flat if ok else tiled).append((it, nb.value, lds.value) if ok else (it, 0, 0))
# ... 27 lines not shown
    def strip_table(self, items, seg=None):
        lib = _lib.load()
        nb = C.c_int()
        buf, block_begin, rows = bytearray(), 0, 0
        plane_at = max_k = 0
        for it in items:
            if seg is None:
                gy, x, z, act, gW, gb, accumulate = it
                M, N = gy.shape
                K = x.shape[1]
                rec = (gy.data_ptr(), x.data_ptr(), z.data_ptr() if z is not None else 0, gW.data_ptr(),
                       gb.data_ptr() if gb is not None else 0, M, N, K, int(accumulate), int(act))
                tail = (0, 0, 0)
                per_rank = 0
            else:
                per_rank, N, K, off_g, off_x, gW, gb, _acc, recv, total = it
                M = seg * per_rank
                rec = (recv.data_ptr() + 4 * off_g, recv.data_ptr() + 4 * off_x, 0, gW.data_ptr(),
                       gb.data_ptr() if gb is not None else 0, M, N, K, int(bool(_acc)), 0)
                tail = (per_rank, total, 0)
            if lib.cgv_wgrad_strip_plan(M, N, K, per_rank, C.byref(nb)) != 0:
                raise RuntimeError(lib.cgv_last_error_string().decode())
            buf += self.RECORD.pack(*rec, block_begin, 0, 0, tail[0], tail[1], plane_at // 256)
            plane_at += int(lib.cgv_wgrad_strip_split_plane_bytes(M, K)) if M <= self.STRIP_SPLIT_MAX_ROWS else 0
            block_begin += nb.value
            rows = max(rows, M)
            max_k = max(max_k, K)
        dev = items[0][0].device if seg is None else items[0][8].device
        self._strip_plan = (plane_at, max_k)
        return self.upload(bytes(buf), dev), block_begin, rows

    STRIP_SPLIT_MAX_ROWS = 96
    STRIP_SPLIT_MIN_ROWS = 64
    _strip_ws = {}
    _strip_captured = []

    def strip_launch(self, table, n_problems, blocks, rows, tag):
        from .options import HOST
        plane_bytes, max_k = self._strip_plan
        if (HOST["strip_split"] and self.STRIP_SPLIT_MIN_ROWS <= rows <= self.STRIP_SPLIT_MAX_ROWS and plane_bytes > 0) or HOST["strip_split"] == 2:
            dev = table.device
            ws = self._strip_ws.get(dev)
            if ws is None or ws.numel() < plane_bytes:
                ws = self._strip_ws[dev] = torch.empty(max(plane_bytes, 32 << 20), dtype=torch.uint8, device=dev)
            if torch.cuda.is_current_stream_capturing() and not any(t is ws for t in self._strip_captured):
                self._strip_captured.append(ws)
            _lib.call("cgv_grouped_wgrad_strip_split", _lib.ptr(table), n_problems, blocks, rows, max_k, _lib.ptr(ws), ws.numel(),
                      _lib.stream_ptr(), tag=tag)
        else:
            _lib.call("cgv_grouped_wgrad_strip", _lib.ptr(table), n_problems, blocks, rows, _lib.stream_ptr(), tag=tag)

    def launch(self, items):
        if not items:
            return
        lib = _lib.load()
        assert lib.cgv_wgrad_record_bytes() == self.RECORD.size
        if len(items) > self.MAX_PROBLEMS:
            raise RuntimeError("too many queued weight-gradient problems")
        strips = [it for it in items if self.strip_rows(it[0].shape[0], it[0].shape[1], it[1].shape[1])]
        ids = {id(it) for it in strips}
        small = [it for it in items if id(it) not in ids and self.kernel != "mfma"
                 and lib.cgv_skinny_supported(it[0].shape[0], it[0].shape[1], it[1].shape[1])]
        ids |= {id(it) for it in small}
        large = [it for it in items if id(it) not in ids]
        dev = items[0][0].device
        tk, tw, nb = C.c_int(), C.c_int(), C.c_int()
        if small:
            table, block_begin, max_lds = self.small_table(small)
            _lib.call("cgv_grouped_wgrad", _lib.ptr(table), len(small), block_begin, max_lds, _lib.stream_ptr(),
                      tag="grouped_wgrad")
        if strips:
            table, block_begin, rows = self.strip_table(strips)
            self.strip_launch(table, len(strips), block_begin, rows, "grouped_wgrad_strip")
        if large:
            buf, block_begin = bytearray(), 0
            from .options import HOST
            split = HOST["wgrad_split"] == 1
            tile = 128 if split else wgrad_tile([(gy.shape[0], gy.shape[1], x.shape[1]) for gy, x, *_rest in large])
            for gy, x, z, act, gW, gb, accumulate in large:
                M, N = gy.shape
                K = x.shape[1]
                if lib.cgv_wgrad_gathered_plan_tile(M, N, K, 0, tile, C.byref(tk), C.byref(nb)) != 0:
                    raise RuntimeError(lib.cgv_last_error_string().decode())
                buf += self.RECORD.pack(gy.data_ptr(), x.data_ptr(), z.data_ptr() if z is not None else 0, gW.data_ptr(),
                                        gb.data_ptr() if gb is not None else 0, M, N, K, int(accumulate), int(act),
                                        block_begin, tk.value, 0, 0, 0, 0)
                block_begin += nb.value
            table = self.upload(bytes(buf), dev)
            if split:
                _lib.call("cgv_grouped_wgrad_split", _lib.ptr(table), len(large), block_begin, _lib.stream_ptr(),
                          tag="grouped_wgrad_tiles")
            else:
                _lib.call("cgv_grouped_wgrad_gathered_tile", _lib.ptr(table), len(large), block_begin, tile, _lib.stream_ptr(),
                          tag="grouped_wgrad_tiles")


class _QueueScope:
    def __init__(self, q):
        self.q = q

    def __enter__(self):
        self.q.active = True
        self.q.items = []
        self.q.filters = []
        return self.q

    def __exit__(self, *exc):
        self.q.active = False


wgrad_queue = WeightGradQueue()


def _claim_producer(producer, consumer):
    import weakref
    prev = getattr(producer, "_cgv_claim", None)
    if prev is None:
        producer._cgv_claim = weakref.ref(consumer)
        return producer
    first = prev() if callable(prev) else None
    if first is not None:
        first.producer = None
    producer._cgv_claim = False
    return None


class _LinearFn(torch.autograd.Function):

    @staticmethod
    def forward(ctx, x, weight, bias, act, fork=False, slot=None, producer=None):
        y = _LinearFn._forward(ctx, x, weight, bias, act)
        ctx.set_materialize_grads(False)
        ctx.slot = slot
        ctx.producer = None
        if (producer is not None and HOST_OPTION("act_downstream") and x.grad_fn is producer and ctx.mode in ("tile", "skinny")
                and getattr(producer, "act", ACT_NONE) != ACT_NONE and getattr(producer, "mode", None) == ctx.mode):
            ctx.producer = _claim_producer(producer, ctx)
        if slot is not None:
            slot.armed = True
        if fork:
            return y, x.view_as(x)
        return y

    @staticmethod
    def _forward(ctx, x, weight, bias, act):
        x2 = x.reshape(-1, x.shape[-1])
        ctx.params = (weight, bias)
        ctx.act = act
        ctx.mode = _gemm_mode(x2, weight, bias)
        ctx.bias_aligned = bias is None or bias.data_ptr() % 16 == 0
        N = weight.shape[0]
        x2 = x2.contiguous()
        if x2.data_ptr() % 16:
            x2 = x2.clone()
        M, K = x2.shape
        y = torch.empty(M, N, dtype=torch.float32, device=x.device)
        z = torch.empty_like(y) if act else None
        _lib.call(FWD_ENTRY[fwd_choice(M, N, K, ctx.bias_aligned)], _lib.ptr(x2), _lib.ptr(weight), _lib.ptr(bias), _lib.ptr(y),
                  _lib.ptr(z), M, N, K, act, _lib.stream_ptr())
        ctx.save_for_backward(x2, weight, z)
        return y.reshape(x.shape[:-1] + (N,))

    @staticmethod
    def backward(ctx, gy, g_alias=None):
        if gy is None:
            if ctx.needs_input_grad[1]:
                zero_unreached(ctx.params)
            return _LinearFn._with_parked(ctx, g_alias), None, None, None, None, None, None
        out = _LinearFn._backward(ctx, gy, g_alias)
        return out + (None, None, None)

    @staticmethod
    def _with_parked(ctx, gx):
        slot = getattr(ctx, "slot", None)
        if slot is None:
            return gx
        slot.linear_done = True
        g = slot.take()
        if g is None:
            return gx
        spread = slot.broadcast(g)
        return spread.reshape(gx.shape) + gx if gx is not None else spread.reshape(ctx.saved_tensors[0].shape)

    @staticmethod
    def _backward(ctx, gy, add):
        gx, gw, gb, _none = _LinearFn._backward_core(ctx, gy, add)
        if getattr(ctx, "slot", None) is not None and ctx.needs_input_grad[0]:
            gx = _LinearFn._with_parked(ctx, gx)
        return gx, gw, gb, None

    @staticmethod
    def _backward_core(ctx, gy, add):
        x, weight, z = ctx.saved_tensors
        w_param, b_param = ctx.params
        act = ctx.act
        if getattr(ctx, "act_done", False):
            ctx.act_done = False
            act = ACT_NONE
        add2 = add.reshape(-1, add.shape[-1]) if add is not None else None
        if add2 is not None and not (add2.is_contiguous() and add2.data_ptr() % 16 == 0 and add2.dtype == torch.float32):
            add2 = add2.contiguous().float()
        need_x, need_w = ctx.needs_input_grad[0], ctx.needs_input_grad[1]
        need_b = b_param is not None and ctx.needs_input_grad[2]
        gy2 = gy.reshape(-1, gy.shape[-1]).contiguous()
        M, K = x.shape
        N = weight.shape[0]
        gx = None
        if ctx.mode == "tile":
            if gy2.data_ptr() % 16:
                gy2 = gy2.clone()
            if not (need_w and wgrad_queue.active and _is_direct(w_param) and w_param.grad.is_contiguous()
                    and (not need_b or (_is_direct(b_param) and b_param.grad.is_contiguous())) and lib_has_rows(M, N, K)):
                return _LinearFn._backward_prepared(ctx, gy, gy2, add, act, need_x, need_w, need_b)
        if need_x:
            gx = torch.empty(M, K, dtype=torch.float32, device=gy.device)
            kind = bwd_input_choice(M, N, K, _lib.split_workspace_ready(), ctx.bias_aligned, gy2.data_ptr() % 16 == 0)
            slot = getattr(ctx, "slot", None)
            g = slot.g if (slot is not None and ctx.mode == "tile" and kind == "tile") else None
            parked = None
            if g is not None and (g.dtype == torch.float32 and g.is_contiguous() and g.data_ptr() % 16 == 0 and g.dim() == 2
                                  and g.shape[1] == K and slot.mapping.numel() == M):
                parked = slot.take()
            fused = bwd_input_launch(kind, gy2, z, act, weight, gx, add2, slot, parked, getattr(ctx, "producer", None))
            gx = gx.reshape(gy.shape[:-1] + (K,))
            if add is not None and not fused:
                gx = gx + add.reshape(gx.shape)
        gw = gb = None
        if need_w:
            gw, gb = wgrad_sink(w_param, b_param, gy2, x, z, act, (M, N, K), like=weight, need_b=need_b)
        return (gx if need_x else add), gw, gb, None

    @staticmethod
    def _backward_prepared(ctx, gy, gy2, add, act, need_x, need_w, need_b):
        x, weight, z = ctx.saved_tensors
        w_param, b_param = ctx.params
        M, K = x.shape
        N = weight.shape[0]
        st = _lib.stream_ptr()
        gx = gw = None
        if need_w:
            w_param._cgv_rank = (M, N, K)
        g2 = torch.empty_like(gy2) if act != ACT_NONE else gy2
        tb, acc_b, gb = _grad_target(b_param, b_param) if need_b else (None, False, None)
        if act != ACT_NONE or need_b:
            _lib.call("cgv_dense_grad_prepare", _lib.ptr(gy2), _lib.ptr(z), _lib.ptr(g2) if act != ACT_NONE else None,
                      _lib.ptr(tb), M, N, act, int(acc_b), st)
        if need_x:
            gx = torch.empty(M, K, dtype=torch.float32, device=gy.device)
            _lib.call("cgv_tile_linear_bwd_input", _lib.ptr(g2), _lib.ptr(weight), _lib.ptr(gx), M, N, K, st)
            gx = gx.reshape(gy.shape[:-1] + (K,))
            if add is not None:
                gx = gx + add.reshape(gx.shape)
        if need_w:
            tw, acc_w, gw = _grad_target(w_param, weight)
            if wgrad_queue.active and gw is None and lib_has_rows(M, N, K):
                wgrad_queue.enqueue(g2, x, None, ACT_NONE, tw, None, acc_w)
            else:
                _lib.call("cgv_tile_linear_wgrad", _lib.ptr(g2), _lib.ptr(x), _lib.ptr(tw), M, N, K, int(acc_w), st)
        return (gx if need_x else add), gw, gb, None


class _PairLinearFn(torch.autograd.Function):

    @staticmethod
    def forward(ctx, x_a, x_b, w_a, b_a, w_b, b_b, act_a, act_b):
        xa = x_a.reshape(-1, x_a.shape[-1]).contiguous()
        xb = xa if x_b is x_a else x_b.reshape(-1, x_b.shape[-1]).contiguous()
        M, K = xa.shape
        N = w_a.shape[0]
        ya, yb = torch.empty(M, N, dtype=torch.float32, device=xa.device), torch.empty(M, N, dtype=torch.float32, device=xa.device)
        za = torch.empty_like(ya) if act_a else None
        zb = torch.empty_like(yb) if act_b else None
        _lib.call("cgv_pair_linear_fwd", _lib.ptr(xa), _lib.ptr(xb), _lib.ptr(w_a), _lib.ptr(w_b), _lib.ptr(b_a), _lib.ptr(b_b),
                  _lib.ptr(ya), _lib.ptr(yb), _lib.ptr(za), _lib.ptr(zb), int(act_a), int(act_b), M, N, K, _lib.stream_ptr())
        ctx.params = (w_a, b_a, w_b, b_b)
        ctx.acts = (int(act_a), int(act_b))
        ctx.same_x = x_b is x_a
        ctx.save_for_backward(xa, xb, w_a, w_b, za, zb)
        return ya.reshape(x_a.shape[:-1] + (N,)), yb.reshape(x_b.shape[:-1] + (N,))

    @staticmethod
    def backward(ctx, g_a, g_b):
        xa, xb, wa, wb, za, zb = ctx.saved_tensors
        pa_w, pa_b, pb_w, pb_b = ctx.params
        act_a, act_b = ctx.acts
        M, K = xa.shape
        N = wa.shape[0]
        ga = (g_a if g_a is not None else torch.zeros(M, N, dtype=torch.float32, device=xa.device)).reshape(M, N).contiguous()
        gb = (g_b if g_b is not None else torch.zeros(M, N, dtype=torch.float32, device=xa.device)).reshape(M, N).contiguous()
        need_xa, need_xb = ctx.needs_input_grad[0], ctx.needs_input_grad[1]
        gxa = gxb = None
        if need_xa or need_xb:
            lib = _lib.load()
            nbytes = 2 * int(lib.cgv_skinny_bwd_input_workspace_bytes(M, N, K)) or 2 * 4 * M * K
            nbytes = max(nbytes, 2 * 4 * M * K)
            ws = torch.empty(nbytes, dtype=torch.uint8, device=xa.device)
            gxa = torch.empty(M, K, dtype=torch.float32, device=xa.device)
            gxb = None if ctx.same_x else torch.empty(M, K, dtype=torch.float32, device=xa.device)
            _lib.call("cgv_pair_linear_bwd_input", _lib.ptr(ga), _lib.ptr(gb), _lib.ptr(za), _lib.ptr(zb), _lib.ptr(wa), _lib.ptr(wb),
                      act_a, act_b, _lib.ptr(gxa), _lib.ptr(gxb), M, N, K, ws.data_ptr(), nbytes, _lib.stream_ptr())
        grads_w = []
        for g2, x2, z, act, w_param, b_param, need_w, need_b in (
                (ga, xa, za, act_a, pa_w, pa_b, ctx.needs_input_grad[2], pa_b is not None and ctx.needs_input_grad[3]),
                (gb, xb, zb, act_b, pb_w, pb_b, ctx.needs_input_grad[4], pb_b is not None and ctx.needs_input_grad[5])):
            grads_w += wgrad_sink(w_param, b_param, g2, x2, z, act, (M, N, K), need_b=need_b) if need_w else (None, None)
        shape_a = None if gxa is None else gxa.reshape(xa.shape)
        return (shape_a if need_xa else None, (gxb if need_xb else None), grads_w[0], grads_w[1], grads_w[2], grads_w[3], None, None)


class _TilePairFn(torch.autograd.Function):

    @staticmethod
    def forward(ctx, x_a, x_b, w_a, b_a, w_b, b_b, acts, slot, producer=None):
        same = x_b is x_a
        ctx.producer = None
        if (producer is not None and not same and HOST_OPTION("act_downstream") and getattr(producer, "acts", None) is not None
                and x_a.grad_fn is producer and x_b.grad_fn is producer and all(a != ACT_NONE for a in producer.acts)):
            ctx.producer = _claim_producer(producer, ctx)
        act_a, act_b = int(acts[0]), int(acts[1])
        xa = x_a.reshape(-1, x_a.shape[-1]).contiguous()
        xb = xa if same else x_b.reshape(-1, x_b.shape[-1]).contiguous()
        M, K = xa.shape
        N = w_a.shape[0]
        new = lambda: torch.empty(M, N, dtype=torch.float32, device=xa.device)
        ya, yb = new(), new()
        za, zb = (new() if act_a else None), (new() if act_b else None)
        _lib.call("cgv_tile_pair_linear_fwd", _lib.ptr(xa), _lib.ptr(w_a), _lib.ptr(b_a), _lib.ptr(ya), _lib.ptr(za), _lib.ptr(xb),
                  _lib.ptr(w_b), _lib.ptr(b_b), _lib.ptr(yb), _lib.ptr(zb), M, N, K, act_a, act_b, _lib.stream_ptr())
        ctx.params, ctx.acts, ctx.same, ctx.slot = (w_a, b_a, w_b, b_b), (act_a, act_b), same, slot
        if slot is not None:
            slot.armed = True
        ctx.save_for_backward(xa, xb, w_a, w_b, za, zb)
        ctx.set_materialize_grads(False)
        return ya.reshape(x_a.shape[:-1] + (N,)), yb.reshape(x_b.shape[:-1] + (N,)), x_a.view_as(x_a)

    @staticmethod
    def backward(ctx, g_a, g_b, g_alias):
        xa, xb, wa, wb, za, zb = ctx.saved_tensors
        pa_w, pa_b, pb_w, pb_b = ctx.params
        (act_a, act_b), slot = ctx.acts, ctx.slot
        done = getattr(ctx, "act_done", (False, False))
        ctx.act_done = (False, False)
        act_a = ACT_NONE if done[0] else act_a
        act_b = ACT_NONE if done[1] else act_b
        M, K = xa.shape
        N = wa.shape[0]
        st = _lib.stream_ptr()
        prep = lambda g: None if g is None else g.reshape(M, N).contiguous()
        ga, gb = prep(g_a), prep(g_b)
        new = lambda: torch.empty(M, K, dtype=torch.float32, device=xa.device)
        kind = bwd_input_choice(M, N, K, _lib.split_workspace_ready(), long_row_split=False)

        def single(g, z, w, add, act, parked=None):
            gx = new()
            bwd_input_launch(kind, g, z, act, w, gx, add, slot, parked)
            return gx
        gxa = gxb = None
        need_a, need_b = ctx.needs_input_grad[0], ctx.needs_input_grad[1]
        if ctx.same:
            if need_a:
                add = None if g_alias is None else g_alias.reshape(M, K).contiguous()
                parked = None
                if slot is not None:
                    slot.linear_done = True
                    parked = slot.take()
                par_ok = parked is None or (parked.dtype == torch.float32 and parked.is_contiguous() and parked.shape[1] == K
                                            and parked.data_ptr() % 16 == 0)
                if (ga is not None and gb is not None and par_ok and HOST_OPTION("pair_sum2")
                        and (add is None or (add.dtype == torch.float32 and add.data_ptr() % 16 == 0))):
                    gxa = new()
                    _lib.call("cgv_tile_linear_bwd_input_sum2", _lib.ptr(ga), _lib.ptr(za) if act_a != ACT_NONE else None, _lib.ptr(wa),
                              _lib.ptr(gb), _lib.ptr(zb) if act_b != ACT_NONE else None, _lib.ptr(wb), _lib.ptr(add), _lib.ptr(parked),
                              _lib.ptr(slot.mapping) if parked is not None else None,
                              _lib.ptr(slot.plan.rowptr_d) if parked is not None else None, int(slot.mean) if parked is not None else 0,
                              _lib.ptr(gxa), M, N, K, act_a, act_b, st)
                    parked = None
                    gb_done = True
                else:
                    gb_done = False
                if not gb_done and gb is not None:
                    add = single(gb, zb, wb, add, act_b)
                if gb_done:
                    pass
                elif ga is not None and parked is not None and parked.dtype == torch.float32 and parked.is_contiguous() and parked.shape[1] == K:
                    gxa = single(ga, za, wa, add, act_a, parked)
                else:
                    gxa = single(ga, za, wa, add, act_a) if ga is not None else add
                    if parked is not None:
                        spread = slot.broadcast(parked)
                        gxa = spread if gxa is None else gxa + spread
                if gxa is not None:
                    gxa = gxa.reshape(xa.shape)
        else:
            if ga is not None and gb is not None and need_a and need_b:
                gxa, gxb = new(), new()
                prod = ctx.producer
                if prod is not None:
                    pz = prod.saved_tensors
                    _lib.call("cgv_tile_pair_linear_bwd_input_out", _lib.ptr(ga), _lib.ptr(za) if act_a != ACT_NONE else None, _lib.ptr(wa),
                              None, _lib.ptr(gxa), _lib.ptr(gb), _lib.ptr(zb) if act_b != ACT_NONE else None, _lib.ptr(wb), None,
                              _lib.ptr(gxb), M, N, K, act_a, act_b, _lib.ptr(pz[4]), int(prod.acts[0]), _lib.ptr(pz[5]),
                              int(prod.acts[1]), st)
                    prod.act_done = (True, True)
                else:
                    _lib.call("cgv_tile_pair_linear_bwd_input", _lib.ptr(ga), _lib.ptr(za) if act_a != ACT_NONE else None, _lib.ptr(wa), None,
                              _lib.ptr(gxa), _lib.ptr(gb), _lib.ptr(zb) if act_b != ACT_NONE else None, _lib.ptr(wb), None, _lib.ptr(gxb),
                              M, N, K, act_a, act_b, st)
            else:
                gxa = single(ga, za, wa, None, act_a) if (ga is not None and need_a) else None
                gxb = single(gb, zb, wb, None, act_b) if (gb is not None and need_b) else None
        grads_w = []
        for g2, x2, z, act, w_param, b_param, need_w, need_bias in (
                (ga, xa, za, act_a, pa_w, pa_b, ctx.needs_input_grad[2], pa_b is not None and ctx.needs_input_grad[3]),
                (gb, xb, zb, act_b, pb_w, pb_b, ctx.needs_input_grad[4], pb_b is not None and ctx.needs_input_grad[5])):
            gw = gbias = None
            if need_w and g2 is None:
                zero_unreached((w_param, b_param))
            elif need_w:
                gw, gbias = wgrad_sink(w_param, b_param, g2, x2, z, act, (M, N, K), need_b=need_bias)
            grads_w += [gw, gbias]
        return (gxa if need_a else None, None if ctx.same else (gxb if need_b else None), grads_w[0], grads_w[1], grads_w[2], grads_w[3],
                None, None, None)


def _dense_act(layer):
    if not isinstance(layer, Dense) or layer.dropout_rate:
        return None
    if isinstance(layer.activation, Swish):
        return ACT_SWISH
    return ACT_NONE if layer.activation is None else None


def tile_pair_usable_raw(x_a, x_b, w_a, b_a, w_b, b_b) -> bool:
    if not (x_a.is_cuda and x_a.dtype == torch.float32 and x_b.dtype == torch.float32 and b_a is not None and b_b is not None):
        return False
    if w_a.shape != w_b.shape or x_a.shape != x_b.shape or x_a.dim() != 2:
        return False
    M, K = x_a.shape
    N = w_a.shape[0]
    if gemm_mode_or_none(x_a, w_a, b_a)[0] != "tile" or not _lib.load().cgv_tile_pair_supported(M, N, K):
        return False
    tens = (x_a, x_b, w_a, w_b, b_a, b_b)
    return (all(_is_direct(p) and p.grad.is_contiguous() for p in (w_a, w_b, b_a, b_b))
            and all(t.is_contiguous() and t.data_ptr() % 16 == 0 for t in tens) and lib_has_rows(M, N, K))


def tile_pair_usable(x_a, x_b, la, lb) -> bool:
    return (_dense_act(la) is not None and _dense_act(lb) is not None
            and tile_pair_usable_raw(x_a, x_b, la.weight, la.bias, lb.weight, lb.bias))


def tile_pair(x_a, x_b, la, lb, slot=None, producer=None):
    return _TilePairFn.apply(x_a, x_b, la.weight, la.bias, lb.weight, lb.bias, (_dense_act(la), _dense_act(lb)), slot, producer)


def _ptr_table(tensors):
    return (C.c_void_p * len(tensors))(*[(t.data_ptr() if t is not None else None) for t in tensors])


class _MultiLinearFn(torch.autograd.Function):

    @staticmethod
    def forward(ctx, acts, group, *args):
        n = len(acts)
        xs, wb = args[:n], args[n:]
        ws, bs = wb[0::2], wb[1::2]
        x2 = []
        for j, x in enumerate(xs):
            if group == 2 and j % 2 == 1 and x is xs[j - 1]:
                x2.append(x2[-1])
            else:
                x2.append(x.reshape(-1, x.shape[-1]).contiguous())
        M, K = x2[0].shape
        N = ws[0].shape[0]
        dev = x2[0].device
        ys = [torch.empty(M, N, dtype=torch.float32, device=dev) for _ in range(n)]
        zs = [torch.empty(M, N, dtype=torch.float32, device=dev) if acts[j] else None for j in range(n)]
        act_arr = (C.c_int * n)(*[int(a) for a in acts])
        _lib.call("cgv_multi_linear_fwd", n, _ptr_table(x2), _ptr_table(ws), _ptr_table(bs), _ptr_table(ys), _ptr_table(zs),
                  act_arr, M, N, K, _lib.stream_ptr())
        ctx.params = (ws, bs)
        ctx.acts, ctx.group, ctx.n = tuple(int(a) for a in acts), int(group), n
        ctx.shape = xs[0].shape
        ctx.save_for_backward(*x2, *[w for w in ws], *[z if z is not None else x2[0].new_empty(0) for z in zs])
        return tuple(y.reshape(xs[0].shape[:-1] + (N,)) for y in ys)

    @staticmethod
    def backward(ctx, *gys):
        n, group, acts = ctx.n, ctx.group, ctx.acts
        saved = ctx.saved_tensors
        x2, wd, zs = saved[:n], saved[n:2 * n], [z if z.numel() else None for z in saved[2 * n:]]
        pws, pbs = ctx.params
        M, K = x2[0].shape
        N = wd[0].shape[0]
        dev = x2[0].device
        g2 = [(g if g is not None else torch.zeros(M, N, dtype=torch.float32, device=dev)).reshape(M, N).contiguous() for g in gys]
        need_x = [ctx.needs_input_grad[2 + j] for j in range(n)]
        gxs = [None] * n
        if any(need_x):
            lib = _lib.load()
            per = max(int(lib.cgv_skinny_bwd_input_workspace_bytes(M, N, K)), 4 * M * K)
            ws = torch.empty(n * per, dtype=torch.uint8, device=dev)
# ... 60 lines not shown
                or lin.weight.data_ptr() % 16 or (lin.bias is not None and lin.bias.data_ptr() % 16)):
            return None
    hid = _MultiLinearFn.apply(tuple(h[1] for h in heads), 2, *xs, *[t for lin in first for t in (lin.weight, lin.bias)])
    return _MultiLinearFn.apply(tuple(out_acts), 1, *hid, *[t for lin in second for t in (lin.weight, lin.bias)])


def pair_linear_usable(x_a, x_b, lin_a, lin_b) -> bool:
    if not (x_a.is_cuda and x_a.dtype == torch.float32 and x_b.dtype == torch.float32 and x_a.shape == x_b.shape):
        return False
    wa, wb = lin_a.weight, lin_b.weight
    if wa.shape != wb.shape or (lin_a.bias is None) != (lin_b.bias is None):
        return False
    M = x_a.numel() // x_a.shape[-1]
    N, K = wa.shape
    return 1 <= M <= 16 and N % 4 == 0 and K % 4 == 0 and N >= 64 and x_a.shape[-1] == K and wa.is_contiguous() and wb.is_contiguous()


def HOST_OPTION(name):
    from .options import HOST
    return HOST[name]


def dual_heads(head_a, head_b, x, out_act_a: int = ACT_NONE, out_act_b: int = ACT_NONE):
    ma, mb = list(head_a), list(head_b)
    codes = MLPHead._CODES
    if (len(ma) == 3 and len(mb) == 3 and isinstance(ma[0], nn.Linear) and isinstance(mb[0], nn.Linear)
            and type(ma[1]) in codes and type(mb[1]) in codes and isinstance(ma[2], nn.Linear) and isinstance(mb[2], nn.Linear)
            and pair_linear_usable(x, x, ma[0], mb[0])):
        ha, hb = _PairLinearFn.apply(x, x, ma[0].weight, ma[0].bias, mb[0].weight, mb[0].bias, codes[type(ma[1])], codes[type(mb[1])])
        if pair_linear_usable(ha, hb, ma[2], mb[2]):
            return _PairLinearFn.apply(ha, hb, ma[2].weight, ma[2].bias, mb[2].weight, mb[2].bias, out_act_a, out_act_b)
        return linear_fn(ha, ma[2].weight, ma[2].bias, out_act_a), linear_fn(hb, mb[2].weight, mb[2].bias, out_act_b)
    if (len(ma) == 3 and len(mb) == 3 and isinstance(ma[0], nn.Linear) and isinstance(mb[0], nn.Linear) and type(ma[1]) in codes
            and type(mb[1]) in codes and isinstance(ma[2], nn.Linear) and isinstance(mb[2], nn.Linear) and x.dim() == 2
            and x.requires_grad and torch.is_grad_enabled() and HOST_OPTION("head_pairs")
            and tile_pair_usable_raw(x, x, ma[0].weight, ma[0].bias, mb[0].weight, mb[0].bias)):
        ha, hb, _alias = _TilePairFn.apply(x, x, ma[0].weight, ma[0].bias, mb[0].weight, mb[0].bias, (codes[type(ma[1])], codes[type(mb[1])]), None)
        if tile_pair_usable_raw(ha, hb, ma[2].weight, ma[2].bias, mb[2].weight, mb[2].bias):
            ya, yb, _alias = _TilePairFn.apply(ha, hb, ma[2].weight, ma[2].bias, mb[2].weight, mb[2].bias, (int(out_act_a), int(out_act_b)), None)
            return ya, yb
        return linear_fn(ha, ma[2].weight, ma[2].bias, out_act_a), linear_fn(hb, mb[2].weight, mb[2].bias, out_act_b)
    ya, x_alias = head_a(x, out_act=out_act_a, fork=True)
    return ya, head_b(x_alias, out_act=out_act_b)


def wgrad_tile(shapes) -> int:
    from .options import HOST
    return 128 if HOST["wgrad_tile"] == 128 else 64


def lib_has_rows(M, N, K) -> bool:
    return M >= 1 and N >= 4 and K >= 4 and N % 4 == 0 and K % 4 == 0


FWD_ENTRY = {"decoder_dense": "cgv_decoder_dense_fwd", "skinny": "cgv_skinny_linear_fwd", "tile": "cgv_tile_linear_fwd"}


def fwd_choice(M, N, K, bias_aligned=True, decoder_dense=True, wide_tiles=True) -> str:
    lib = _lib.load()
    if lib.cgv_skinny_supported(M, N, K) and bias_aligned:
        if decoder_dense and M <= 16 and N >= 64:
            return "decoder_dense"
        if wide_tiles and M > 32 and N >= 4096 and lib.cgv_tile_supported(M, N, K):
            return "tile"
        return "skinny"
    if M <= 128 and N <= 1200 and bias_aligned and lib.cgv_skinny_fwd_supported(M, N, K):
        return "skinny"
    return "tile"


def bwd_input_choice(M, N, K, split_ready, bias_aligned=True, gy_aligned=True, short_tiles=True, long_row_split=True) -> str:
    lib = _lib.load()
    if lib.cgv_skinny_supported(M, N, K) and bias_aligned:
        if (M > 32 and ((short_tiles and N <= 1024) or (N < 4096 and split_ready)) and gy_aligned
                and lib.cgv_tile_supported(M, N, K)):
            return "tile"
        return "skinny"
    if (long_row_split and M <= 128 and N >= 4096 and lib.cgv_skinny_bwd_input_supported(M, N, K)
            and not (M > 64 and split_ready)):
        return "skinny"
    return "tile"


def bwd_input_launch(kind, gy2, z, act, weight, gx, add=None, slot=None, parked=None, producer=None) -> bool:
    M, K = gx.shape
    N = weight.shape[0]
    z = z if act != ACT_NONE else None
    if kind == "skinny":
        if producer is not None and skinny_bwd_input_out(gy2, z, weight, add, gx, M, N, K, act, producer.saved_tensors[2],
                                                         int(producer.act)):
            producer.act_done = True
            return True
        return skinny_bwd_input(gy2, z, weight, gx, M, N, K, act, add=add)
    st = _lib.stream_ptr()
    P = _lib.ptr
    if parked is not None:
        _lib.call("cgv_tile_linear_bwd_input_act_add_bcast", P(gy2), P(z), P(weight), P(add), P(parked), P(slot.mapping),
                  P(slot.plan.rowptr_d), int(slot.mean), P(gx), M, N, K, act, st)
    elif producer is not None:
        _lib.call("cgv_tile_linear_bwd_input_out", P(gy2), P(z), P(weight), P(add), P(gx), M, N, K, act,
                  P(producer.saved_tensors[2]), int(producer.act), st)
        producer.act_done = True
    elif add is not None:
        _lib.call("cgv_tile_linear_bwd_input_act_add", P(gy2), P(z), P(weight), P(add), P(gx), M, N, K, act, st)
    else:
        _lib.call("cgv_tile_linear_bwd_input_act", P(gy2), P(z), P(weight), P(gx), M, N, K, act, st)
        return False
    return True


def wgrad_sink(w_param, b_param, gy, x, z, act, shape, exch=True, like=None, need_b=True, stacked=None, flush=True):
    w_param._cgv_rank = shape
    if exch:
        w_param._cgv_exch = shape
        if b_param is not None:
            b_param._cgv_exch = shape
    tw, acc_w, gw = _grad_target(w_param, w_param if like is None else like)
    if stacked is not None:
        stacked._cgv_rank = shape
        _tv, acc_v, _ = _grad_target(stacked, stacked)
        if acc_v != acc_w:
            raise RuntimeError("stacked weights of one problem disagree on first-write / accumulate state")
        n, k = w_param.shape
        tw = torch.as_strided(tw, (n + stacked.shape[0], k), (k, 1))
    tb, acc_b, gb = _grad_target(b_param, b_param) if (b_param is not None and need_b) else (None, acc_w, None)
    if acc_b != acc_w:
        raise RuntimeError("weight and bias of one layer disagree on first-write / accumulate state")
    wgrad_queue.enqueue(gy, x, z if act != ACT_NONE else None, act, tw, tb, acc_w)
    if flush and not (wgrad_queue.active and gw is None and gb is None):
        wgrad_queue.flush()
    return gw, gb


def zero_unreached(params):
    for prm in params:
        if _is_direct(prm) and prm._cgv_pending:
            prm.grad.zero_()
            prm._cgv_pending = False


def skinny_bwd_input(gy2, z, weight, gx, M, N, K, act, stream=None, add=None) -> bool:
    lib = _lib.load()
    nbytes = lib.cgv_skinny_bwd_input_workspace_bytes(M, N, K)
    ws = torch.empty(max(nbytes, 16), dtype=torch.uint8, device=gx.device)
    if add is not None and add.is_contiguous() and add.data_ptr() % 16 == 0 and nbytes > 0:
        rc = lib.cgv_skinny_linear_bwd_input_add(_lib.ptr(gy2), _lib.ptr(z) if z is not None else None, _lib.ptr(weight), _lib.ptr(add),
                                                 _lib.ptr(gx), M, N, K, act, ws.data_ptr(), nbytes,
                                                 stream if stream is not None else _lib.stream_ptr())
        if rc == 0:
            return True
        if rc != -2:
            raise RuntimeError(f"cgv_skinny_linear_bwd_input_add failed with code {rc}: {lib.cgv_last_error_string().decode()}")
    _lib.call("cgv_skinny_linear_bwd_input", _lib.ptr(gy2), _lib.ptr(z) if z is not None else None, _lib.ptr(weight),
              _lib.ptr(gx), M, N, K, act, ws.data_ptr(), nbytes, stream if stream is not None else _lib.stream_ptr())
    return False


def skinny_bwd_input_out(gy2, z, weight, add, gx, M, N, K, act, z_out, act_out) -> bool:
    lib = _lib.load()
    nbytes = lib.cgv_skinny_bwd_input_workspace_bytes(M, N, K)
    if nbytes <= 0 or (add is not None and not (add.is_contiguous() and add.data_ptr() % 16 == 0)) or z_out.data_ptr() % 16:
        return False
    ws = torch.empty(nbytes, dtype=torch.uint8, device=gx.device)
    rc = lib.cgv_skinny_linear_bwd_input_out(_lib.ptr(gy2), _lib.ptr(z) if z is not None else None, _lib.ptr(weight), _lib.ptr(add),
                                             _lib.ptr(gx), M, N, K, act, _lib.ptr(z_out), int(act_out), ws.data_ptr(), nbytes,
                                             _lib.stream_ptr())
    if rc == 0:
        return True
    if rc != -2:
        raise RuntimeError(f"cgv_skinny_linear_bwd_input_out failed with code {rc}: {lib.cgv_last_error_string().decode()}")
    return False


def _is_direct(param):
    return param is not None and getattr(param, "_cgv_direct", False) and param.grad is not None


def _grad_target(param, like):
    if _is_direct(param) and param.grad.is_contiguous():
        acc = not param._cgv_pending
        param._cgv_pending = False
        return param.grad, acc, None
    out = torch.empty_like(like)
    return out, False, out


def _direct_grad(param, write_into, compute):
    if _is_direct(param):
        if param._cgv_pending:
            write_into(param.grad)
            param._cgv_pending = False
        else:
            param.grad.add_(compute())
        return None
    return compute()


def mark_direct_grad(*params):
    for p in params:
        if p is not None:
            p._cgv_direct_ok = True


class _DirectSink(torch.autograd.Function):

    @staticmethod
    def forward(ctx, param):
        ctx.param = param
        return param.view_as(param)

    @staticmethod
    def backward(ctx, g):
        return _direct_grad(ctx.param, lambda t: t.copy_(g.reshape(t.shape)), lambda: g)

# ... 124 lines not shown
```

### coarsegrainingvae_amd/train.py

```python
from __future__ import annotations

import sys
from typing import Optional

import numpy as np
import torch
from torch import nn

from .data import batch_to, prepare_batch
from .model import CGequiVAE, CGprior, EquiEncoder, EquivariantPsuedoDecoder
from .primitives import Linear, MLPHead

EPS = 1e-6
CLIP_NORM = 0.01
optim_dict = {"adam": torch.optim.Adam, "sgd": torch.optim.SGD}


def KL(mu1, std1, mu2, std2):
    if mu2 is None:
        return -0.5 * torch.sum(1 + torch.log(std1.pow(2)) - mu1.pow(2) - std1.pow(2), dim=-1).mean()
    return 0.5 * ((std1.pow(2) / std2.pow(2)).sum(-1) + ((mu1 - mu2).pow(2) / std2).sum(-1)
                  + torch.log(std2.pow(2)).sum(-1) - torch.log(std1.pow(2)).sum(-1) - std1.shape[-1]).mean()


def loss_terms(out, batch, beta, gamma):
    S_mu, S_sigma, H_prior_mu, H_prior_sigma, xyz, xyz_recon = out
    if S_mu is not None and H_prior_mu is not None and xyz_recon.is_cuda:
        from . import ops
        loss, terms = ops.elbo_loss(S_mu, S_sigma, H_prior_mu, H_prior_sigma, xyz, xyz_recon, batch["bond_edge_list"],
                                    beta, gamma)
        return loss, terms[1], terms[2], terms[3]
    if xyz_recon.is_cuda:
        from . import ops
        ops.materialise_reconstruct(xyz_recon)
    loss_kl = KL(S_mu, S_sigma, H_prior_mu, H_prior_sigma) if S_mu is not None else xyz.new_zeros(())
    loss_recon = (xyz_recon - xyz).pow(2).mean()
    if gamma != 0.0:
        e = batch["bond_edge_list"]
        gen_dist = ((xyz_recon[e[:, 0]] - xyz_recon[e[:, 1]]).pow(2).sum(-1) + EPS).sqrt()
        data_dist = ((xyz[e[:, 0]] - xyz[e[:, 1]]).pow(2).sum(-1) + EPS).sqrt()
        loss_graph = (gen_dist - data_dist).pow(2).mean()
    else:
        loss_graph = xyz.new_zeros(())
    return loss_recon + loss_kl * beta + loss_graph * gamma, loss_kl, loss_recon, loss_graph


def build_model(n_basis, n_rbf, atom_cutoff, cg_cutoff, enc_nconv, dec_nconv, n_cgs, activation="swish",
                det=False, invariantdec=False, cg_mp=False, seed: Optional[int] = 123):
    if seed is not None:
        torch.manual_seed(seed)
    atom_mu = MLPHead(Linear(n_basis, n_basis), nn.ReLU(), Linear(n_basis, n_basis))
    atom_sigma = MLPHead(Linear(n_basis, n_basis), nn.ReLU(), Linear(n_basis, n_basis))
    decoder = EquivariantPsuedoDecoder(n_atom_basis=n_basis, n_rbf=n_rbf, cutoff=atom_cutoff, num_conv=dec_nconv,
                                       activation=activation, breaksym=(n_cgs == 3))
    encoder = EquiEncoder(n_conv=enc_nconv, n_atom_basis=n_basis, n_rbf=n_rbf, cutoff=cg_cutoff,
                          activation=activation, cg_mp=cg_mp, dir_mp=False)
    prior = CGprior(n_conv=enc_nconv, n_atom_basis=n_basis, n_rbf=n_rbf, cutoff=cg_cutoff, activation=activation,
                    dir_mp=False)
    return CGequiVAE(encoder, decoder, atom_mu, atom_sigma, n_cgs, feature_dim=n_basis, prior_net=prior, det=det,
                     equivariant=not invariantdec)


def train_step(model, batch, optimizer, beta, gamma, eps=None, train=True, grad_sync=None):
    out = model(batch, eps=eps) if eps is not None else model(batch)
    loss, kl, recon, graph = loss_terms(out, batch, beta, gamma)
    decision = loss.detach() if grad_sync is None else grad_sync.mean_scalar(loss.detach())
    lv = float(decision)
    skipped = lv >= gamma * 200.0 or lv != lv
    if not skipped:
        if train:
            optimizer.zero_grad(set_to_none=True)
            loss.backward()
            if grad_sync is not None:
                grad_sync.all_reduce(model)
            torch.nn.utils.clip_grad_norm_(model.parameters(), CLIP_NORM)
            optimizer.step()
        else:
            loss.backward()
    return loss.detach(), kl.detach(), recon.detach(), graph.detach(), skipped, out


def loop(loader, optimizer, device, model, beta, epoch, gamma, eta=0.0, kappa=0.0, train=True, looptext="",
         tqdm_flag=True, grad_sync=None):
    totals, kls, recons, graphs = [], [], [], []
    model.train()
    mode = "{} {}".format(looptext, "train" if train else "valid")
    if tqdm_flag:
        from tqdm import tqdm
        loader = tqdm(loader, position=0, file=sys.stdout, leave=True, desc="({} epoch #{})".format(mode, epoch))
    xyz = xyz_recon = None
    postfix = []
    for batch in loader:
        if "_graph" not in batch:
            batch = prepare_batch(batch, device)
        else:
            batch = batch_to(batch, device)
        loss, kl, recon, graph, skipped, out = train_step(model, batch, optimizer, beta, gamma, train=train,
                                                          grad_sync=grad_sync)
        xyz, xyz_recon = out[4], out[5]
        kls.append(kl.item())
        if skipped:
            print(loss.item())
            continue
        recons.append(recon.item())
        graphs.append(graph.item())
        totals.append(loss.item())
        memory = torch.cuda.memory_allocated(device) / (1024 ** 2) if torch.cuda.is_available() else 0.0
        postfix = ["total={:.3f}".format(np.mean(totals)), "KL={:.4f}".format(np.mean(kls)),
                   "recon={:.4f}".format(np.mean(recons)), "graph={:.4f}".format(np.mean(graphs)),
                   "memory ={:.4f} Mb".format(memory)]
        if tqdm_flag:
            loader.set_postfix_str(" ".join(postfix))
    for result in postfix:
        print(result)
    mean = lambda a: float(np.mean(a)) if a else float("nan")
    return mean(totals), mean(kls), mean(recons), mean(graphs), xyz, xyz_recon
```

### include/cgvae_hip.h

```cpp
#ifndef CGVAE_HIP_H
#define CGVAE_HIP_H

#include <stddef.h>
#include <stdint.h>

#ifdef __cplusplus
extern "C" {
#endif

#define CGV_VERSION 101

#define CGV_E_BADARG (-1)
#define CGV_E_UNSUPPORTED (-2)
#define CGV_E_WORKSPACE (-3)

int cgv_version(void);
const char* cgv_last_error_string(void);

enum {
  CGV_OPT_MSG_FWD_SPLIT = 0,
  CGV_OPT_MSG_BWD_SPLIT = 1,
  CGV_OPT_CSR_BUILD = 2,
  CGV_OPT_PSEUDO_CHUNKS = 3,
  CGV_OPT_WGRAD_TILING = 4,
// ... 165 lines not shown
                          int K, int act, void* stream);
int cgv_decoder_uv_fwd(const float* rows, const float* Wuv, float* UV, float* stack, int n_nodes, int n_feat, void* stream);
int cgv_decoder_gate_fwd(const float* a0, const float* W1p, const float* b1p, const float* UV, const float* stack,
                         const float* v2, float* a, float* s3, float* v3, int n_nodes, int n_feat, void* stream);
int cgv_decoder_gate_bwd(const float* UV, const float* a, const float* gs_base , const float* gs_slices ,
                         int gs_n_slices, int64_t gs_slice_stride, const float* gv , const float* W1p, float* ga,
                         float* gUV, float* gs_sum, float* slices_out, int64_t out_slice_stride, int n_nodes, int n_feat,
                         void* stream);
int cgv_decoder_dense_bwd(const float* g_slices, int g_n_slices, int64_t g_slice_stride, const float* z , int act,
                          const float* W, float* g_dense, float* slices_out, int64_t out_slice_stride, int n_nodes, int N, int K,
                          void* stream);
int cgv_decoder_uv_bwd(const float* gstack_slices, int n_slices, int64_t slice_stride, const float* UV, const float* stack,
                       const float* gs_res, const float* Wuv, const float* gUV, float* gUV_out, float* g_s2, float* slices_out,
                       int64_t out_slice_stride, int n_nodes, int n_feat, void* stream);
int cgv_decoder_msg_bwd(const float* phi, const float* s, const float* sbar, const float* v, const float* vbar,
                        const float* geom_d, const int32_t* rowptr_d, const int32_t* src_d, const float* geom_s,
                        const int32_t* rowptr_s, const int32_t* dst_s, const float* Wd, const float* bd, const float* gh,
                        const float* ghb , const float* gvrows_slices, int n_slices, int64_t slice_stride,
                        const float* gv_res , const float* gvb , const float* W2, float* g_phi, float* g_s,
                        float* g_sbar, float* g_v, float* g_vbar, float* gWd, float* gbd, float* slices_out,
                        int64_t out_slice_stride, int n_nodes, int n_feat, int n_rbf, int n_edges, void* stream);
int cgv_decoder_slices_to_dense(const float* base , const float* slices, int n_slices, int64_t slice_stride,
                                float* out, int n_nodes, int n_feat, void* stream);

int cgv_update_rows_from_vec(const float* v , float* rows , int n_nodes, int n_feat, void* stream);
int cgv_update_vec_from_rows(const float* rows, const float* res , float* vec, int n_nodes, int n_feat,
                             void* stream);
int cgv_update_norm_stack_fwd(const float* s , const float* Vv, float* stack , int n_nodes, int n_feat,
                              int ld, void* stream);
int cgv_update_norm_stack_bwd(const float* gstack, const float* Vv, const float* stack, const float* g_res ,
                              float* g_s, float* gVv, int n_nodes, int n_feat, int ld, int accumulate, void* stream);
int cgv_update_gate_fwd(const float* U, const float* Vv, const float* a, const float* s_res ,
                        const float* v_res , float* ds , float* dv ,
                        int n_nodes, int n_feat, int ld, void* stream);
int cgv_update_gate_bwd(const float* U, const float* Vv, const float* a, const float* g_ds, const float* g_dv,
                        float* gU, float* gVv, float* ga, int n_nodes, int n_feat, int ld, void* stream);

int cgv_skinny_max_rows(void);
int cgv_skinny_supported(int M, int N, int K);
int cgv_skinny_fwd_supported(int M, int N, int K);
int cgv_skinny_linear_fwd(const float* x, const float* W, const float* bias, float* y, float* z , int M, int N,
                          int K, int act, void* stream);
int cgv_skinny_bwd_input_supported(int M, int N, int K);
size_t cgv_skinny_bwd_input_workspace_bytes(int M, int N, int K);
int cgv_skinny_linear_bwd_input(const float* gy, const float* z , const float* W, float* gx, int M, int N, int K,
                                int act, void* ws , size_t ws_bytes, void* stream);
int cgv_skinny_linear_bwd_input_add(const float* gy, const float* z , const float* W, const float* add, float* gx,
                                    int M, int N, int K, int act, void* workspace, size_t workspace_bytes, void* stream);
int cgv_skinny_linear_bwd_input_out(const float* gy, const float* z , const float* W, const float* add ,
                                    float* gx, int M, int N, int K, int act, const float* z_out, int act_out, void* workspace,
                                    size_t workspace_bytes, void* stream);
int cgv_dense_grad_prepare(const float* gy, const float* z , float* g_out , float* gb ,
                           int M, int N, int act, int accumulate, void* stream);
int cgv_tile_supported(int M, int N, int K);
int cgv_tile_linear_fwd(const float* x, const float* W, const float* bias , float* y, float* z , int M,
                        int N, int K, int act, void* stream);
int cgv_tile_linear_bwd_input(const float* g, const float* W, float* gx, int M, int N, int K, void* stream);
int cgv_tile_linear_bwd_input_act(const float* gy, const float* z , const float* W, float* gx, int M, int N, int K,
                                  int act, void* stream);
int cgv_tile_linear_bwd_input_act_add(const float* gy, const float* z , const float* W, const float* add, float* gx,
                                      int M, int N, int K, int act, void* stream);
int cgv_tile_linear_bwd_input_act_add_bcast(const float* gy, const float* z, const float* W, const float* add, const float* seg_grad,
                                            const int64_t* row2seg, const int32_t* seg_rowptr, int mean, float* gx, int M, int N,
                                            int K, int act, void* stream);

int cgv_tile_pair_supported(int M, int N, int K);
int cgv_tile_pair_linear_fwd(const float* x_a, const float* W_a, const float* bias_a, float* y_a, float* z_a, const float* x_b,
                             const float* W_b, const float* bias_b, float* y_b, float* z_b, int M, int N, int K, int act_a,
                             int act_b, void* stream);
int cgv_tile_pair_linear_bwd_input(const float* gy_a, const float* z_a, const float* W_a, const float* add_a, float* gx_a,
                                   const float* gy_b, const float* z_b, const float* W_b, const float* add_b, float* gx_b, int M,
                                   int N, int K, int act_a, int act_b, void* stream);
int cgv_tile_linear_bwd_input_norm_stack(const float* gy, const float* z, const float* W, int M, int N, int K, int act,
                                         const float* stack, const float* Vv, const float* g_res, float* g_s, float* gVv, int ld,
                                         int accumulate, void* stream);
int cgv_tile_bwd_input_plan(int M, int N, int K, int np, int* shares , int* streamk );
int cgv_tile_bwd_input_split(void* workspace, size_t workspace_bytes, void* stream);
int cgv_tile_linear_bwd_input_out(const float* gy, const float* z, const float* W, const float* add, float* gx, int M, int N,
                                  int K, int act, const float* z_out, int act_out, void* stream);
int cgv_tile_pair_linear_bwd_input_out(const float* gy_a, const float* z_a, const float* W_a, const float* add_a, float* gx_a,
                                       const float* gy_b, const float* z_b, const float* W_b, const float* add_b, float* gx_b,
                                       int M, int N, int K, int act_a, int act_b, const float* z_out_a, int act_out_a,
                                       const float* z_out_b, int act_out_b, void* stream);
int cgv_tile_linear_bwd_input_sum2(const float* gy_a, const float* z_a, const float* W_a, const float* gy_b, const float* z_b,
                                   const float* W_b, const float* add, const float* seg_grad, const int64_t* row2seg,
                                   const int32_t* seg_rowptr, int mean, float* gx, int M, int N, int K, int act_a, int act_b,
                                   void* stream);
int cgv_tile_linear_wgrad(const float* g, const float* x, float* gW, int M, int N, int K, int accumulate, void* stream);
int cgv_wgrad_record_bytes(void);
int cgv_wgrad_plan(int M, int N, int K, int* tiles_k , int* tile_w , int* n_blocks );
int cgv_wgrad_lds_floats(int M, int tile_w);
int cgv_grouped_wgrad(const void* table_dev, int n_problems, int total_blocks, int max_lds_floats, void* stream);
int cgv_wgrad_gathered_plan(int M, int N, int K, int seg_rows, int* tiles_k , int* n_blocks );
int cgv_grouped_wgrad_gathered(const void* table_dev, int n_problems, int total_blocks, void* stream);
int cgv_wgrad_gathered_plan_tile(int M, int N, int K, int seg_rows, int tile, int* tiles_k , int* n_blocks );
int cgv_grouped_wgrad_gathered_tile(const void* table_dev, int n_problems, int total_blocks, int tile, void* stream);
int cgv_grouped_wgrad_split(const void* table_dev, int n_problems, int total_blocks, void* stream);
int cgv_grouped_wgrad_gathered_sumsq(const void* table_dev, int n_problems, int total_blocks, double* partial, double* sumsq,
                                     void* stream);
int cgv_grouped_wgrad_gathered_adam(const void* table_dev, int n_problems, int total_blocks, const float* arena_g,
                                    float* arena_p, float* arena_m, float* arena_v, float lr, float beta1, float beta2,
                                    float eps, const float* state, void* stream);
int cgv_wgrad_strip_max_rows(void);
int cgv_wgrad_strip_plan(int M, int N, int K, int seg_rows, int* n_blocks );
int cgv_grouped_wgrad_strip(const void* table_dev, int n_problems, int total_blocks, int max_rows, void* stream);
int cgv_wgrad_strip_split_max_rows(void);
size_t cgv_wgrad_strip_split_plane_bytes(int M, int K);
int cgv_grouped_wgrad_strip_split(const void* table_dev, int n_problems, int total_blocks, int max_rows, int max_k, void* ws,
                                  size_t ws_bytes, void* stream);
int cgv_grouped_wgrad_strip_sumsq(const void* table_dev, int n_problems, int total_blocks, int max_rows, double* partial,
                                  double* sumsq, void* stream);
int cgv_grouped_wgrad_strip_adam(const void* table_dev, int n_problems, int total_blocks, int max_rows, const float* arena_g,
                                 float* arena_p, float* arena_m, float* arena_v, float lr, float beta1, float beta2,
                                 float eps, const float* state, void* stream);
int cgv_pack_record_bytes(void);
int cgv_pack_plan(int M, int N, int K, int* n_blocks );
int cgv_pack_operands(const void* table_dev, int n_problems, int total_blocks, void* stream);

int cgv_reconstruct_fwd(const float* v, const float* cg_xyz, const int32_t* rowptr, const int32_t* atom, const int64_t* chan,
                        int n_beads, int n_feat, int offset, float* xyz , void* stream);
int cgv_reconstruct_bwd(const float* g_xyz, const int32_t* rowptr, const int32_t* atom, const int64_t* chan, int n_beads,
                        int n_feat, int offset, float* g_v, float* g_cg_xyz , void* stream);

size_t cgv_elbo_workspace_bytes(int n_beads, int n_feat);
int cgv_elbo_fwd(const float* mu, const float* sigma, const float* prior_mu, const float* prior_std, const float* xyz,
                 const float* xyz_recon, const int64_t* bonds, int n_beads, int n_feat, int n_atoms, int n_bonds,
                 float beta, float gamma, float* out4, float* loss_out ,
                 float* g_mu, float* g_sigma, float* g_prior_mu, float* g_prior_std, float* g_xyz_recon,
                 void* workspace , size_t workspace_bytes, void* stream);
int cgv_elbo_scale(const float* g_loss, float* g_mu, float* g_sigma, float* g_prior_mu, float* g_prior_std, int n_bead_elems,
                   float* g_xyz_recon, int n_atom_elems, void* stream);
int cgv_loss_tail_supported(int n_beads, int n_feat, int n_atoms, int n_bonds);
size_t cgv_loss_tail_workspace_bytes(int n_beads);
int cgv_loss_tail(const float* V, const float* cg_xyz, const int32_t* rowptr, const int32_t* atom_of, const int32_t* bead_of,
                  const int64_t* chan, const float* mu, const float* sigma, const float* prior_mu, const float* prior_std,
                  const float* xyz, const int64_t* bonds, int n_beads, int n_feat, int n_atoms, int n_bonds, int offset,
                  float beta, float gamma, float* xyz_recon, float* out4, float* loss_out, float* g_mu, float* g_sigma,
                  float* g_prior_mu, float* g_prior_std, float* g_xyz_recon, float* g_V, void* workspace, size_t workspace_bytes,
                  void* stream);

int cgv_optim_state_floats(void);
int cgv_optim_partial_floats(void);
int cgv_adam_clip_step(float* p, const float* g, float* m, float* v, int64_t n, float lr, float beta1, float beta2,
                       float eps, float max_norm, float grad_scale, const float* loss ,
                       float skip_threshold, float* state, float* partial, void* stream);
int cgv_optim_prepare(const float* g, int64_t n, float beta1, float beta2, float max_norm, float grad_scale,
                      const float* loss , float skip_threshold, float* state, float* partial,
                      void* stream);
int cgv_adam_apply(float* p, const float* g, float* m, float* v, int64_t n, float lr, float beta1, float beta2, float eps,
                   const float* state, void* stream);
int cgv_sgd_apply(float* p, const float* g, int64_t n, float lr, const float* state, void* stream);

int cgv_wgrad_gram(const void* table_dev, int n_problems, int max_rows, double* sumsq, void* workspace,
                   size_t workspace_bytes, void* stream);
size_t cgv_wgrad_gram_workspace_bytes(int n_problems);
int cgv_wgrad_gram_mfma(const void* table_dev, int n_problems, int max_rows, double* sumsq, void* workspace,
                        size_t workspace_bytes, void* stream);
size_t cgv_wgrad_gram_mfma_workspace_bytes(int n_problems, int max_rows);
int cgv_wgrad_gram_mfma_max_rows(void);
int cgv_rank_update_supported(int M, int N, int K);
int cgv_optim_prepare_extra(const float* g, int64_t n, const double* extra, int n_extra, float beta1, float beta2,
                            float max_norm, float grad_scale, const float* loss, float skip_threshold, float* state,
                            float* partial, void* stream);
int cgv_grouped_wgrad_adam(const void* table_dev, int n_problems, int total_blocks, int max_lds_floats,
                           const float* arena_g, float* arena_p, float* arena_m, float* arena_v, float lr, float beta1,
                           float beta2, float eps, const float* state, void* stream);
// ... 230 lines not shown
```

Before: 1298.

## Skip dead gradient columns in backward input and weight-gradient GEMMs

Tags upstream gradients whose nonzero values sit in a known column window, for example from slicing. The backward-input tile GEMM then restricts its reduction to that window, and the gathered wgrad kernel only computes live row tiles, writing zeros (or leaving accumulators unchanged) for dead tiles. This avoids multiply-adds and loads on columns known to be zero. It adds a thread-local pending-window protocol and record fields that could go stale, and it depends on a host option and on whether producers mark gradients.

Result: faster. 1315, median of 4 (+1.3%).

```diff
diff --git a/coarsegrainingvae_amd/_lib.py b/coarsegrainingvae_amd/_lib.py
--- a/coarsegrainingvae_amd/_lib.py
+++ b/coarsegrainingvae_amd/_lib.py
@@ -123,6 +123,10 @@
     "cgv_tile_bwd_input_split": (_i, [_p, _sz, _p]),
     "cgv_tile_pair_linear_bwd_input_out": (_i, [_p] * 10 + [_i, _i, _i, _i, _i, _p, _i, _p, _i, _p]),
     "cgv_tile_linear_bwd_input_sum2": (_i, [_p] * 10 + [_i, _p, _i, _i, _i, _i, _i, _p]),
+    "cgv_tile_bwd_input_window": (_i, [_i, _i, _i]),
+    "cgv_tile_bwd_input_plan_win": (_i, [_i, _i, _i, _i, _i, _i, _p, _p]),
+    "cgv_tile_linear_bwd_input_win": (_i, [_p] * 5 + [_i, _i, _i, _i, _p, _i, _i, _i, _p]),
+    "cgv_tile_pair_linear_bwd_input_win": (_i, [_p] * 10 + [_i, _i, _i, _i, _i, _p, _i, _p, _i, _i, _i, _p]),
     "cgv_segment_reduce2": (_i, [_p, _i, _p, _p, _i, _p, _p, _p, _i, _i, _p]),
     "cgv_skinny_linear_bwd_input_add": (_i, [_p, _p, _p, _p, _p, _i, _i, _i, _i, _p, _sz, _p]),
     "cgv_skinny_linear_bwd_input_out": (_i, [_p] * 5 + [_i, _i, _i, _i, _p, _i, _p, _sz, _p]),
@@ -397,4 +401,6 @@
     ktimer.end(tok)
     if rc != 0:
         msg = lib.cgv_last_error_string().decode("utf-8", "replace")
+        if name.startswith("cgv_tile_") and "bwd_input" in name:
+            lib.cgv_tile_bwd_input_window(0, -1, 0)
         raise RuntimeError(f"{name} failed with code {rc}: {msg}")
diff --git a/coarsegrainingvae_amd/csrc/tile_gemm.hip b/coarsegrainingvae_amd/csrc/tile_gemm.hip
--- a/coarsegrainingvae_amd/csrc/tile_gemm.hip
+++ b/coarsegrainingvae_amd/csrc/tile_gemm.hip
@@ -404,6 +404,7 @@
 struct OutAct { const float* z; int act; const float* z2; int act2; };
 struct SplitN { float* part; unsigned* ticket; int n; };
 struct NormStackOut { const float* stack; const float* Vv; const float* g_res; float* g_s; float* gVv; int F; int ld; int accumulate; };
+struct BwdWindow { int k0, kn; };
 struct BcastAdd {
   const float* src;
   const int64_t* row2seg;
@@ -424,7 +425,9 @@
                                                         BwdSource more = BwdSource{nullptr, nullptr, nullptr, 0},
                                                         OutAct oa = OutAct{nullptr, 0, nullptr, 0},
                                                         SplitN sp = SplitN{nullptr, nullptr, 1},
-                                                        NormStackOut ns = NormStackOut{nullptr, nullptr, nullptr, nullptr, nullptr, 0, 0, 0}) {
+                                                        NormStackOut ns = NormStackOut{nullptr, nullptr, nullptr, nullptr, nullptr, 0, 0, 0},
+                                                        BwdWindow win = BwdWindow{0, -1}) {
+  const int n_lo = win.kn < 0 ? 0 : win.k0, n_hi = win.kn < 0 ? N : win.k0 + win.kn;
   if (blockIdx.z) { g = s2.g; W = s2.W; gx = s2.gx; z = s2.z; add = s2.add; act = s2.act; bc.src = nullptr; oa.z = oa.z2; oa.act = oa.act2; }
   __shared__ float red[WAVES][MB * 4][4][64];
   const int lane = threadIdx.x & 63;
@@ -451,7 +454,8 @@
   const int steps_all = (N + 15) / 16, zper = (steps_all + sp.n - 1) / sp.n;
   const int z_beg = min(zs * zper, steps_all), steps = min(z_beg + zper, steps_all);
   const int per = (steps - z_beg + WAVES - 1) / WAVES;
-  const int st_beg = min(z_beg + wave * per, steps), st_end = min(st_beg + per, steps);
+  const int st_all = min(z_beg + wave * per, steps);
+  const int st_beg = min(max(st_all, n_lo / 16), steps), st_end = min(min(st_all + per, steps), (n_hi + 15) / 16);
   constexpr int SB = WAVES >= 16 ? 3 : 2;
   const float* wcol = W + (kok ? kcol : 0);
   ptrdiff_t zo = zoff;
@@ -469,8 +473,8 @@
 #pragma unroll
     for (int u = 0; u < SB; ++u) {
       const int n = 16 * (st0 + u);
-      const bool in = st0 + u < st_end && n + 4 * q < N;
-      const int ng = in ? n : -4 * q, nw = in ? n + 4 * q : 0;
+      const bool in = st0 + u < st_end && n + 4 * q >= n_lo && n + 4 * q < n_hi;
+      const int ng = in ? n : n_lo - 4 * q, nw = in ? n + 4 * q : n_lo;
 #pragma unroll
       for (int mb = 0; mb < MB; ++mb) {
         B.a[u][mb] = *reinterpret_cast<const float4*>(gr[mb] + ng);
@@ -484,7 +488,7 @@
 #pragma unroll
     for (int u = 0; u < SB; ++u) {
       if (st0 + u >= st_end) break;
-      const bool nok = 16 * (st0 + u) + 4 * q < N;
+      const bool nok = 16 * (st0 + u) + 4 * q >= n_lo && 16 * (st0 + u) + 4 * q < n_hi;
 #pragma unroll
       for (int mb = 0; mb < MB; ++mb) {
         float4 av = B.a[u][mb];
@@ -852,16 +856,37 @@
 }
 }
 
+static int window_ok(int N, int k0, int kn) {
+  return k0 >= 0 && kn >= 4 && (k0 % 4) == 0 && (kn % 4) == 0 && (int64_t)k0 + kn <= N;
+}
+namespace cgv {
+struct PendingWindow { BwdWindow win; int N; };
+static thread_local PendingWindow g_next_window = {{0, -1}, 0};
+}
+
 static int tile_bwd_input_launch(const float* g, const float* z, int act, const float* W, float* gx, int M, int N, int K,
                                  void* stream, const char* what, const float* add = nullptr,
                                  cgv::BcastAdd bc = cgv::BcastAdd{nullptr, nullptr, nullptr, 0},
                                  const cgv::BwdSecond* second = nullptr,
                                  cgv::BwdSource more = cgv::BwdSource{nullptr, nullptr, nullptr, 0},
                                  cgv::OutAct oa = cgv::OutAct{nullptr, 0, nullptr, 0},
-                                 cgv::NormStackOut ns = cgv::NormStackOut{nullptr, nullptr, nullptr, nullptr, nullptr, 0, 0, 0}) {
+                                 cgv::NormStackOut ns = cgv::NormStackOut{nullptr, nullptr, nullptr, nullptr, nullptr, 0, 0, 0},
+                                 cgv::BwdWindow win = cgv::BwdWindow{0, -1}) {
   hipStream_t st = (hipStream_t)stream;
   const cgv::BwdSecond s2 = second ? *second : cgv::BwdSecond{nullptr, nullptr, nullptr, nullptr, nullptr, 0};
   const unsigned np = second ? 2u : 1u;
+  if (win.kn < 0 && cgv::g_next_window.win.kn >= 0) {
+    const cgv::PendingWindow pend = cgv::g_next_window;
+    if (pend.N != N || !window_ok(N, pend.win.k0, pend.win.kn)) {
+      cgv::g_next_window = cgv::PendingWindow{{0, -1}, 0};
+      cgv::set_error("%s: the announced window [%d, %d) of %d columns does not fit this launch (N = %d)", what, pend.win.k0,
+                     pend.win.k0 + pend.win.kn, pend.N, N);
+      return CGV_E_BADARG;
+    }
+    win = pend.win;
+  }
+  cgv::g_next_window = cgv::PendingWindow{{0, -1}, 0};
+  if (win.kn == N) win = cgv::BwdWindow{0, -1};
   const cgv::BwdInputChoice choice = cgv::bwd_input_choice(M, N, K, (int)np, cgv::sk_ws_ready(stream));
   if (const int bpc = choice.bpc;
       bpc != 0 && !ns.stack && act == 0 && (!more.g || more.act == 0) && (!second || s2.act == 0) &&
@@ -883,10 +908,10 @@
   const int kt = (K + 63) / 64;
   switch (choice.kernel) {
     case cgv::BWD_R32_W8:
-      hipLaunchKernelGGL((cgv::tile_bwd_input_k<2, 8>), dim3(kt, (M + 31) / 32, np), dim3(512), 0, st, g, W, gx, M, N, K, z, act, add, bc, s2, more, oa, cgv::SplitN{nullptr, nullptr, 1}, ns);
+      hipLaunchKernelGGL((cgv::tile_bwd_input_k<2, 8>), dim3(kt, (M + 31) / 32, np), dim3(512), 0, st, g, W, gx, M, N, K, z, act, add, bc, s2, more, oa, cgv::SplitN{nullptr, nullptr, 1}, ns, win);
       break;
     case cgv::BWD_R32_W4:
-      hipLaunchKernelGGL((cgv::tile_bwd_input_k<2, 4>), dim3(kt, (M + 31) / 32, np), dim3(256), 0, st, g, W, gx, M, N, K, z, act, add, bc, s2, more, oa, cgv::SplitN{nullptr, nullptr, 1}, ns);
+      hipLaunchKernelGGL((cgv::tile_bwd_input_k<2, 4>), dim3(kt, (M + 31) / 32, np), dim3(256), 0, st, g, W, gx, M, N, K, z, act, add, bc, s2, more, oa, cgv::SplitN{nullptr, nullptr, 1}, ns, win);
       break;
     case cgv::BWD_R16_W16: {
       cgv::SplitN sp{nullptr, nullptr, 1};
@@ -899,11 +924,11 @@
         sp.n = choice.shares;
       }
       hipLaunchKernelGGL((cgv::tile_bwd_input_k<1, 16>), dim3(kt, ((M + 15) / 16) * sp.n, np), dim3(1024), 0, st, g, W, gx, M, N, K, z, act,
-                         add, bc, s2, more, oa, sp, ns);
+                         add, bc, s2, more, oa, sp, ns, win);
       break;
     }
     case cgv::BWD_R16_W8:
-      hipLaunchKernelGGL((cgv::tile_bwd_input_k<1, 8>), dim3(kt, (M + 15) / 16, np), dim3(512), 0, st, g, W, gx, M, N, K, z, act, add, bc, s2, more, oa, cgv::SplitN{nullptr, nullptr, 1}, ns);
+      hipLaunchKernelGGL((cgv::tile_bwd_input_k<1, 8>), dim3(kt, (M + 15) / 16, np), dim3(512), 0, st, g, W, gx, M, N, K, z, act, add, bc, s2, more, oa, cgv::SplitN{nullptr, nullptr, 1}, ns, win);
       break;
   }
   return cgv::check_launch(what);
@@ -1039,6 +1064,60 @@
                                cgv::OutAct{z_out_a, z_out_a ? act_out_a : 0, z_out_b, z_out_b ? act_out_b : 0});
 }
 
+int cgv_tile_bwd_input_window(int k0, int kn, int N) {
+  if (kn < 0) { cgv::g_next_window = cgv::PendingWindow{{0, -1}, 0}; return 0; }
+  CGV_REQUIRE(N >= 4 && (N % 4) == 0 && window_ok(N, k0, kn), "window must lie inside [0, N) with k0 % 4 == 0, kn % 4 == 0, kn >= 4");
+  cgv::g_next_window = cgv::PendingWindow{{k0, kn}, N};
+  return 0;
+}
+
+int cgv_tile_bwd_input_plan_win(int M, int N, int K, int np, int k0, int kn, int* shares, int* streamk) {
+  CGV_REQUIRE(shares && streamk && np >= 1 && np <= 2, "bad argument");
+  CGV_REQUIRE(cgv_tile_supported(M, N, K), "unsupported shape (need N % 4 == 0, K % 4 == 0)");
+  CGV_REQUIRE(window_ok(N, k0, kn), "window must lie inside [0, N) with k0 % 4 == 0, kn % 4 == 0, kn >= 4");
+  const cgv::BwdInputChoice c = cgv::bwd_input_choice(M, N, K, np, true);
+  *streamk = c.bpc != 0;
+  *shares = c.bpc != 0 ? 1 : c.shares;
+  return 0;
+}
+
+int cgv_tile_linear_bwd_input_win(const float* gy, const float* z, const float* W, const float* add, float* gx, int M, int N,
+                                  int K, int act, const float* z_out, int act_out, int k0, int kn, void* stream) {
+  CGV_REQUIRE(gy && W && gx, "null pointer");
+  CGV_REQUIRE(act == 0 || (act >= 1 && act <= cgv::CGV_ACT_MAX && z), "act != 0 needs the saved pre-activation z");
+  CGV_REQUIRE(!z_out || (act_out >= 1 && act_out <= cgv::CGV_ACT_MAX), "z_out needs its activation code");
+  CGV_REQUIRE(cgv_tile_supported(M, N, K), "unsupported shape (need N % 4 == 0, K % 4 == 0)");
+  CGV_REQUIRE(window_ok(N, k0, kn), "window must lie inside [0, N) with k0 % 4 == 0, kn % 4 == 0, kn >= 4");
+  CGV_REQUIRE(((((uintptr_t)gy | (uintptr_t)z | (uintptr_t)W | (uintptr_t)gx | (uintptr_t)add | (uintptr_t)z_out)) & 15) == 0,
+              "operands must be 16-byte aligned");
+  return tile_bwd_input_launch(gy, act ? z : nullptr, act, W, gx, M, N, K, stream, "cgv_tile_linear_bwd_input_win", add,
+                               cgv::BcastAdd{nullptr, nullptr, nullptr, 0}, nullptr, cgv::BwdSource{nullptr, nullptr, nullptr, 0},
+                               cgv::OutAct{z_out, z_out ? act_out : 0, nullptr, 0},
+                               cgv::NormStackOut{nullptr, nullptr, nullptr, nullptr, nullptr, 0, 0, 0}, cgv::BwdWindow{k0, kn});
+}
+
+int cgv_tile_pair_linear_bwd_input_win(const float* gy_a, const float* z_a, const float* W_a, const float* add_a, float* gx_a,
+                                       const float* gy_b, const float* z_b, const float* W_b, const float* add_b, float* gx_b,
+                                       int M, int N, int K, int act_a, int act_b, const float* z_out_a, int act_out_a,
+                                       const float* z_out_b, int act_out_b, int k0, int kn, void* stream) {
+  const int act = act_a;
+  CGV_REQUIRE(gy_a && W_a && gx_a && gy_b && W_b && gx_b && gx_a != gx_b, "null pointer / aliased outputs");
+  CGV_REQUIRE((act_a == 0 || (act_a >= 1 && act_a <= cgv::CGV_ACT_MAX && z_a)) && (act_b == 0 || (act_b >= 1 && act_b <= cgv::CGV_ACT_MAX && z_b)),
+              "act != 0 needs the saved pre-activation");
+  CGV_REQUIRE((!z_out_a || (act_out_a >= 1 && act_out_a <= cgv::CGV_ACT_MAX)) && (!z_out_b || (act_out_b >= 1 && act_out_b <= cgv::CGV_ACT_MAX)),
+              "z_out needs its activation code");
+  CGV_REQUIRE(cgv_tile_supported(M, N, K), "unsupported shape (need N % 4 == 0, K % 4 == 0)");
+  CGV_REQUIRE(window_ok(N, k0, kn), "window must lie inside [0, N) with k0 % 4 == 0, kn % 4 == 0, kn >= 4");
+  CGV_REQUIRE(((((uintptr_t)gy_a | (uintptr_t)z_a | (uintptr_t)W_a | (uintptr_t)gx_a | (uintptr_t)add_a | (uintptr_t)gy_b |
+                 (uintptr_t)z_b | (uintptr_t)W_b | (uintptr_t)gx_b | (uintptr_t)add_b | (uintptr_t)z_out_a | (uintptr_t)z_out_b)) & 15) == 0,
+              "operands must be 16-byte aligned");
+  const cgv::BwdSecond s2{gy_b, W_b, gx_b, act_b ? z_b : nullptr, add_b, act_b};
+  return tile_bwd_input_launch(gy_a, act ? z_a : nullptr, act, W_a, gx_a, M, N, K, stream, "cgv_tile_pair_linear_bwd_input_win", add_a,
+                               cgv::BcastAdd{nullptr, nullptr, nullptr, 0}, &s2, cgv::BwdSource{nullptr, nullptr, nullptr, 0},
+                               cgv::OutAct{z_out_a, z_out_a ? act_out_a : 0, z_out_b, z_out_b ? act_out_b : 0},
+                               cgv::NormStackOut{nullptr, nullptr, nullptr, nullptr, nullptr, 0, 0, 0}, cgv::BwdWindow{k0, kn});
+}
+
 int cgv_tile_linear_wgrad(const float* g, const float* x, float* gW, int M, int N, int K, int accumulate, void* stream) {
   CGV_REQUIRE(g && x && gW, "null pointer");
   CGV_REQUIRE(cgv_tile_supported(M, N, K), "unsupported shape (need N % 4 == 0, K % 4 == 0)");
diff --git a/coarsegrainingvae_amd/csrc/wgrad_gathered.hip b/coarsegrainingvae_amd/csrc/wgrad_gathered.hip
--- a/coarsegrainingvae_amd/csrc/wgrad_gathered.hip
+++ b/coarsegrainingvae_amd/csrc/wgrad_gathered.hip
@@ -539,8 +539,12 @@
   const int lo = wg_find_problem(table, n_problems, item);
   const WgradProblem pr = table[lo];
   const int local = item - pr.block_begin;
-  const int nb = local / pr.tiles_k, kt = local - nb * pr.tiles_k;
   const int M = pr.M, N = pr.N, K = pr.K;
+  const int live0 = wg_live_row0(pr), live1 = live0 + wg_live_rows(pr);
+  const int first_live = live0 / 128, n_live = (live1 + 127) / 128 - first_live;
+  const int rt = local / pr.tiles_k, kt = local - rt * pr.tiles_k;
+  const int dead = rt - n_live;
+  const int nb = rt < n_live ? first_live + rt : (dead < first_live ? dead : dead + n_live);
   const int sr = pr.seg_rows > 0 ? pr.seg_rows : M;
   const int n0 = nb * 128, k0 = kt * 128;
   const int lane = threadIdx.x & 63;
@@ -548,14 +552,33 @@
   const int wn = wave >> 1, wk = wave & 1;
   const int i = lane & 15, q = lane >> 4;
   typedef float f32x4 __attribute__((ext_vector_type(4)));
+  if (rt >= n_live) {
+    const int kcol = k0 + 64 * wk + 4 * i;
+    if (kcol < K) {
+#pragma unroll
+      for (int t = 0; t < 4; ++t)
+#pragma unroll
+        for (int r = 0; r < 4; ++r) {
+          const int row = n0 + 64 * wn + 16 * t + 4 * q + r;
+          if (row >= N) continue;
+          float* dst = pr.gW + (size_t)row * K + kcol;
+          float4 o = make_float4(0.f, 0.f, 0.f, 0.f);
+          if (pr.accumulate) { const float4 old = ldg4_global(dst); o.x += old.x; o.y += old.y; o.z += old.z; o.w += old.w; }
+          stg4_global(dst, o);
+        }
+    }
+    const int n = n0 + (int)threadIdx.x;
+    if (pr.gb && kt == 0 && threadIdx.x < 128 && n < N) pr.gb[n] = pr.accumulate ? pr.gb[n] + 0.f : 0.f;
+    return;
+  }
   f32x4 acc[4][4];
 #pragma unroll
   for (int t = 0; t < 4; ++t)
 #pragma unroll
     for (int c = 0; c < 4; ++c) acc[t][c] = f32x4{0.f, 0.f, 0.f, 0.f};
   const int c4 = 8 * wave + (lane & 7), rq = lane >> 3;
-  const bool gcol = n0 + 4 * c4 < N, xcol = k0 + 4 * c4 < K;
-  const int gcol_at = gcol ? n0 + 4 * c4 : 0, xcol_at = xcol ? k0 + 4 * c4 : 0;
+  const bool gcol = n0 + 4 * c4 < N && n0 + 4 * c4 >= live0 && n0 + 4 * c4 < live1, xcol = k0 + 4 * c4 < K;
+  const int gcol_at = gcol ? n0 + 4 * c4 : live0, xcol_at = xcol ? k0 + 4 * c4 : 0;
   const float* zsrc = pr.act ? pr.z : pr.gy;
   float4 gq[4], zq[4], xq[4];
   float bs[4] = {0.f, 0.f, 0.f, 0.f};
diff --git a/coarsegrainingvae_amd/csrc/wgrad_record.h b/coarsegrainingvae_amd/csrc/wgrad_record.h
--- a/coarsegrainingvae_amd/csrc/wgrad_record.h
+++ b/coarsegrainingvae_amd/csrc/wgrad_record.h
@@ -17,8 +17,11 @@
   int seg_rows;
   int seg_stride;
   int pad;
+  unsigned short live_row0_q, live_rows_q;
 };
 static_assert(sizeof(WgradProblem) == 88, "host/device record layout");
+__host__ __device__ inline int wg_live_row0(const WgradProblem& pr) { return pr.live_rows_q ? 4 * (int)pr.live_row0_q : 0; }
+__host__ __device__ inline int wg_live_rows(const WgradProblem& pr) { return pr.live_rows_q ? 4 * (int)pr.live_rows_q : pr.N; }
 __device__ __forceinline__ size_t wg_row(const WgradProblem& pr, int m, int width) {
   if (pr.seg_rows <= 0) return (size_t)m * width;
   const int seg = m / pr.seg_rows;
diff --git a/coarsegrainingvae_amd/ops.py b/coarsegrainingvae_amd/ops.py
--- a/coarsegrainingvae_amd/ops.py
+++ b/coarsegrainingvae_amd/ops.py
@@ -9,7 +9,8 @@
 
 from . import _lib, options
 from .graph import EdgeGeometry, EdgePlan
-from .primitives import FWD_ENTRY, bwd_input_choice, bwd_input_launch, fwd_choice, linear as _linear, wgrad_queue, wgrad_sink
+from .primitives import (FWD_ENTRY, bwd_input_choice, bwd_input_launch, fwd_choice, linear as _linear, mark_live_columns, wgrad_queue,
+                         wgrad_sink)
 
 _F32 = torch.float32
 
@@ -102,6 +103,8 @@
                       plan.n_src, F, geom.n_rbf, plan.n_edges, plan.n_dst, _lib.ptr(ws), ws_bytes, C.byref(nc), C.byref(kl),
                       _lib.stream_ptr(), tag=f"equi_msg_bwd:Nd{plan.n_dst}:E{plan.n_edges}:gv{int(gv is not None)}")
             wgrad_queue.enqueue_filter(ws, nc.value, kl.value, geom.n_rbf, F, gWd, gbd)
+            if kl.value == 1 and options.HOST["live_slice"]:
+                mark_live_columns(g_phi, F, F)
             return g_phi, g_v, ret_W, ret_b, None, None, None, g_sres, g_vres
         _lib.call("cgv_equi_msg_bwd", _lib.ptr(phi), _lib.ptr(v), _lib.ptr(geom.geom_s), _lib.ptr(plan.rowptr_s),
                   _lib.ptr(plan.dst_s), _lib.ptr(Wd), _lib.ptr(bd), _lib.ptr(gs), _lib.ptr(gv), _lib.ptr(g_phi),
diff --git a/coarsegrainingvae_amd/options.py b/coarsegrainingvae_amd/options.py
--- a/coarsegrainingvae_amd/options.py
+++ b/coarsegrainingvae_amd/options.py
@@ -30,6 +30,7 @@
     "baseline_form": 0,
     "align_form": 0,
     "kde_splits": 0,
+    "live_slice": 1,
     "decoder_dense": 0,
 }
 _DEFAULTS = dict(HOST)
diff --git a/coarsegrainingvae_amd/primitives.py b/coarsegrainingvae_amd/primitives.py
--- a/coarsegrainingvae_amd/primitives.py
+++ b/coarsegrainingvae_amd/primitives.py
@@ -68,6 +68,7 @@
 class WeightGradQueue:
 
     RECORD = struct.Struct("<5Q11i4x")
+    RECORD_LIVE = struct.Struct("<5Q11i2H")
     MAX_PROBLEMS = 512
 
     def __init__(self):
@@ -97,7 +98,9 @@
     def collect(self):
         return _QueueScope(self)
 
-    def enqueue(self, gy, x, z, act, gW, gb, accumulate):
+    def enqueue(self, gy, x, z, act, gW, gb, accumulate, live=None):
+        if live is not None:
+            gy._cgv_live_rows = (int(live[0]), int(live[1]))
         self.items.append((gy, x, z, act, gW, gb, accumulate))
 
     def take(self):
@@ -291,9 +294,12 @@
                 K = x.shape[1]
                 if lib.cgv_wgrad_gathered_plan_tile(M, N, K, 0, tile, C.byref(tk), C.byref(nb)) != 0:
                     raise RuntimeError(lib.cgv_last_error_string().decode())
-                buf += self.RECORD.pack(gy.data_ptr(), x.data_ptr(), z.data_ptr() if z is not None else 0, gW.data_ptr(),
-                                        gb.data_ptr() if gb is not None else 0, M, N, K, int(accumulate), int(act),
-                                        block_begin, tk.value, 0, 0, 0, 0)
+                k0, kn = getattr(gy, "_cgv_live_rows", None) or (0, 0)
+                if not (kn > 0 and k0 % 4 == 0 and kn % 4 == 0 and k0 + kn <= N and N < 4 * 65536):
+                    k0 = kn = 0
+                buf += self.RECORD_LIVE.pack(gy.data_ptr(), x.data_ptr(), z.data_ptr() if z is not None else 0, gW.data_ptr(),
+                                             gb.data_ptr() if gb is not None else 0, M, N, K, int(accumulate), int(act),
+                                             block_begin, tk.value, 0, 0, 0, 0, k0 // 4, kn // 4)
                 block_begin += nb.value
             table = self.upload(bytes(buf), dev)
             if split:
@@ -415,6 +421,7 @@
         M, K = x.shape
         N = weight.shape[0]
         gx = None
+        live = live_columns(gy, N) if ctx.mode == "tile" else None
         if ctx.mode == "tile":
             if gy2.data_ptr() % 16:
                 gy2 = gy2.clone()
@@ -430,13 +437,13 @@
             if g is not None and (g.dtype == torch.float32 and g.is_contiguous() and g.data_ptr() % 16 == 0 and g.dim() == 2
                                   and g.shape[1] == K and slot.mapping.numel() == M):
                 parked = slot.take()
-            fused = bwd_input_launch(kind, gy2, z, act, weight, gx, add2, slot, parked, getattr(ctx, "producer", None))
+            fused = bwd_input_launch(kind, gy2, z, act, weight, gx, add2, slot, parked, getattr(ctx, "producer", None), live)
             gx = gx.reshape(gy.shape[:-1] + (K,))
             if add is not None and not fused:
                 gx = gx + add.reshape(gx.shape)
         gw = gb = None
         if need_w:
-            gw, gb = wgrad_sink(w_param, b_param, gy2, x, z, act, (M, N, K), like=weight, need_b=need_b)
+            gw, gb = wgrad_sink(w_param, b_param, gy2, x, z, act, (M, N, K), like=weight, need_b=need_b, live=live)
         return (gx if need_x else add), gw, gb, None
 
     @staticmethod
@@ -556,13 +563,14 @@
         N = wa.shape[0]
         st = _lib.stream_ptr()
         prep = lambda g: None if g is None else g.reshape(M, N).contiguous()
+        live_a, live_b = live_columns(g_a, N), live_columns(g_b, N)
         ga, gb = prep(g_a), prep(g_b)
         new = lambda: torch.empty(M, K, dtype=torch.float32, device=xa.device)
         kind = bwd_input_choice(M, N, K, _lib.split_workspace_ready(), long_row_split=False)
 
-        def single(g, z, w, add, act, parked=None):
+        def single(g, z, w, add, act, parked=None, live=None):
             gx = new()
-            bwd_input_launch(kind, g, z, act, w, gx, add, slot, parked)
+            bwd_input_launch(kind, g, z, act, w, gx, add, slot, parked, live=live)
             return gx
         gxa = gxb = None
         need_a, need_b = ctx.needs_input_grad[0], ctx.needs_input_grad[1]
@@ -604,6 +612,8 @@
             if ga is not None and gb is not None and need_a and need_b:
                 gxa, gxb = new(), new()
                 prod = ctx.producer
+                if live_a is not None and live_a == live_b:
+                    announce_window(live_a, N)
                 if prod is not None:
                     pz = prod.saved_tensors
                     _lib.call("cgv_tile_pair_linear_bwd_input_out", _lib.ptr(ga), _lib.ptr(za) if act_a != ACT_NONE else None, _lib.ptr(wa),
@@ -616,17 +626,17 @@
                               _lib.ptr(gxa), _lib.ptr(gb), _lib.ptr(zb) if act_b != ACT_NONE else None, _lib.ptr(wb), None, _lib.ptr(gxb),
                               M, N, K, act_a, act_b, st)
             else:
-                gxa = single(ga, za, wa, None, act_a) if (ga is not None and need_a) else None
-                gxb = single(gb, zb, wb, None, act_b) if (gb is not None and need_b) else None
+                gxa = single(ga, za, wa, None, act_a, live=live_a) if (ga is not None and need_a) else None
+                gxb = single(gb, zb, wb, None, act_b, live=live_b) if (gb is not None and need_b) else None
         grads_w = []
-        for g2, x2, z, act, w_param, b_param, need_w, need_bias in (
-                (ga, xa, za, act_a, pa_w, pa_b, ctx.needs_input_grad[2], pa_b is not None and ctx.needs_input_grad[3]),
-                (gb, xb, zb, act_b, pb_w, pb_b, ctx.needs_input_grad[4], pb_b is not None and ctx.needs_input_grad[5])):
+        for g2, x2, z, act, w_param, b_param, need_w, need_bias, live in (
+                (ga, xa, za, act_a, pa_w, pa_b, ctx.needs_input_grad[2], pa_b is not None and ctx.needs_input_grad[3], live_a),
+                (gb, xb, zb, act_b, pb_w, pb_b, ctx.needs_input_grad[4], pb_b is not None and ctx.needs_input_grad[5], live_b)):
             gw = gbias = None
             if need_w and g2 is None:
                 zero_unreached((w_param, b_param))
             elif need_w:
-                gw, gbias = wgrad_sink(w_param, b_param, g2, x2, z, act, (M, N, K), need_b=need_bias)
+                gw, gbias = wgrad_sink(w_param, b_param, g2, x2, z, act, (M, N, K), need_b=need_bias, live=live)
             grads_w += [gw, gbias]
         return (gxa if need_a else None, None if ctx.same else (gxb if need_b else None), grads_w[0], grads_w[1], grads_w[2], grads_w[3],
                 None, None, None)
@@ -853,7 +863,7 @@
     return "tile"
 
 
-def bwd_input_launch(kind, gy2, z, act, weight, gx, add=None, slot=None, parked=None, producer=None) -> bool:
+def bwd_input_launch(kind, gy2, z, act, weight, gx, add=None, slot=None, parked=None, producer=None, live=None) -> bool:
     M, K = gx.shape
     N = weight.shape[0]
     z = z if act != ACT_NONE else None
@@ -865,6 +875,8 @@
         return skinny_bwd_input(gy2, z, weight, gx, M, N, K, act, add=add)
     st = _lib.stream_ptr()
     P = _lib.ptr
+    if live is not None:
+        announce_window(live, N)
     if parked is not None:
         _lib.call("cgv_tile_linear_bwd_input_act_add_bcast", P(gy2), P(z), P(weight), P(add), P(parked), P(slot.mapping),
                   P(slot.plan.rowptr_d), int(slot.mean), P(gx), M, N, K, act, st)
@@ -880,7 +892,7 @@
     return True
 
 
-def wgrad_sink(w_param, b_param, gy, x, z, act, shape, exch=True, like=None, need_b=True, stacked=None, flush=True):
+def wgrad_sink(w_param, b_param, gy, x, z, act, shape, exch=True, like=None, need_b=True, stacked=None, flush=True, live=None):
     w_param._cgv_rank = shape
     if exch:
         w_param._cgv_exch = shape
@@ -897,10 +909,31 @@
     tb, acc_b, gb = _grad_target(b_param, b_param) if (b_param is not None and need_b) else (None, acc_w, None)
     if acc_b != acc_w:
         raise RuntimeError("weight and bias of one layer disagree on first-write / accumulate state")
-    wgrad_queue.enqueue(gy, x, z if act != ACT_NONE else None, act, tw, tb, acc_w)
+    wgrad_queue.enqueue(gy, x, z if act != ACT_NONE else None, act, tw, tb, acc_w, live if stacked is None else None)
     if flush and not (wgrad_queue.active and gw is None and gb is None):
         wgrad_queue.flush()
     return gw, gb
+
+
+def mark_live_columns(g, k0, kn):
+    g._cgv_live = (int(k0), int(kn), g._version)
+
+
+def announce_window(live, N):
+    lib = _lib.load()
+    if lib.cgv_tile_bwd_input_window(int(live[0]), int(live[1]), int(N)) != 0:
+        raise RuntimeError("cgv_tile_bwd_input_window: " + lib.cgv_last_error_string().decode("utf-8", "replace"))
+
+
+def live_columns(g, width):
+    tag = getattr(g, "_cgv_live", None) if g is not None else None
+    if tag is None or not HOST_OPTION("live_slice"):
+        return None
+    k0, kn, version = tag
+    if (version != g._version or g.dim() != 2 or g.shape[1] != width or not g.is_contiguous() or g.dtype != torch.float32
+            or k0 < 0 or kn < 4 or k0 % 4 or kn % 4 or k0 + kn > width or kn == width):
+        return None
+    return k0, kn
 
 
 def zero_unreached(params):
diff --git a/coarsegrainingvae_amd/train.py b/coarsegrainingvae_amd/train.py
--- a/coarsegrainingvae_amd/train.py
+++ b/coarsegrainingvae_amd/train.py
@@ -105,7 +105,8 @@
         recons.append(recon.item())
         graphs.append(graph.item())
         totals.append(loss.item())
-        memory = torch.cuda.memory_allocated(device) / (1024 ** 2) if torch.cuda.is_available() else 0.0
+        on_gpu = torch.cuda.is_available() and torch.device(device).type == "cuda"
+        memory = torch.cuda.memory_allocated(device) / (1024 ** 2) if on_gpu else 0.0
         postfix = ["total={:.3f}".format(np.mean(totals)), "KL={:.4f}".format(np.mean(kls)),
                    "recon={:.4f}".format(np.mean(recons)), "graph={:.4f}".format(np.mean(graphs)),
                    "memory ={:.4f} Mb".format(memory)]
diff --git a/include/cgvae_hip.h b/include/cgvae_hip.h
--- a/include/cgvae_hip.h
+++ b/include/cgvae_hip.h
@@ -271,6 +271,14 @@
                                        const float* gy_b, const float* z_b, const float* W_b, const float* add_b, float* gx_b,
                                        int M, int N, int K, int act_a, int act_b, const float* z_out_a, int act_out_a,
                                        const float* z_out_b, int act_out_b, void* stream);
+int cgv_tile_bwd_input_window(int k0, int kn, int N);
+int cgv_tile_bwd_input_plan_win(int M, int N, int K, int np, int k0, int kn, int* shares , int* streamk );
+int cgv_tile_linear_bwd_input_win(const float* gy, const float* z, const float* W, const float* add, float* gx, int M, int N,
+                                  int K, int act, const float* z_out, int act_out, int k0, int kn, void* stream);
+int cgv_tile_pair_linear_bwd_input_win(const float* gy_a, const float* z_a, const float* W_a, const float* add_a, float* gx_a,
+                                       const float* gy_b, const float* z_b, const float* W_b, const float* add_b, float* gx_b,
+                                       int M, int N, int K, int act_a, int act_b, const float* z_out_a, int act_out_a,
+                                       const float* z_out_b, int act_out_b, int k0, int kn, void* stream);
 int cgv_tile_linear_bwd_input_sum2(const float* gy_a, const float* z_a, const float* W_a, const float* gy_b, const float* z_b,
                                    const float* W_b, const float* add, const float* seg_grad, const int64_t* row2seg,
                                    const int32_t* seg_rowptr, int mean, float* gx, int M, int N, int K, int act_a, int act_b,
```
